# byronknoll/cmix

Hardware: AMD Instinct MI355X
Metric: input bytes/s on enwik8 at 1 GPU; compressed-size parity vs CPU ref (higher is better)
Workload: dtype f32

## Files before the change

cmix_amd/csrc/cmx_api.hip:

```cpp
#include <hip/hip_runtime.h>
#include <math.h>
#include <stdio.h>
#include <stdlib.h>
#include <string.h>
#include <stddef.h>
#include <string>
#include <map>
#include <mutex>
#include <vector>

#include "../../include/cmix_amd.h"
#include "mixnet_state.h"
#include "cmx_late.h"
#include "cmx_streams.h"
#include "cmx_verify.h"

extern "C" __global__ void cmx_mixnet_kernel(MixState*, const float*, const uint32_t*,
                                             const uint8_t*, const float*, int, float*, float*, int);
extern "C" __global__ void cmx_mixnet_spec_kernel(MixState*, SpecXfer*, const float*, const uint32_t*, const uint8_t*, const float*, int, float*,
                                                  float*, int);
extern "C" __global__ void cmx_mixnet_spec_jitter_kernel(MixState*, SpecXfer*, const float*, const uint32_t*, const uint8_t*, const float*, int, float*, float*, int);
extern "C" __global__ void cmx_mixnet_spec_late_kernel(MixState*, SpecXfer*, const float*, const uint32_t*, const float*, int, float*, float*, int, CmxLate);
extern "C" __global__ void cmx_mixnet_spec_verify_kernel(MixState*, SpecXfer*, const float*, const uint32_t*, const uint8_t*, const float*, int, float*, float*, int,
                                                         CmxVerify);
extern "C" __global__ void cmx_mixnet_verify_kernel(const MixState*, const float*, const uint32_t*, const uint8_t*, const float*, int, CmxVerify);
extern "C" __global__ void cmx_mixnet_verify_fold_kernel(CmxVerifyHdr*, unsigned long long, int);
extern "C" __global__ void cmx_mixnet_verify_xor_kernel(void*, int, unsigned);
extern "C" __global__ void cmx_sse_init_kernel(MixState*);
extern "C" __global__ void cmx_probe_libm_kernel(int, const float*, float*, size_t);

namespace {

thread_local std::string g_err;
void set_err(const std::string& s) { g_err = s; }

#define HIP_OK(call)                                                                  \
  do {                                                                                \
    hipError_t e_ = (call);                                                           \
    if (e_ != hipSuccess) {                                                           \
      set_err(std::string(#call) + ": " + hipGetErrorString(e_));                     \
      return fail_value;                                                              \
    }                                                                                 \
  } while (0)

const float kLr[CMX_MIXERS] = {
    0.005f, 0.0005f, 0.005f, 0.0005f, 0.005f, 0.002f, 0.002f, 0.005f, 0.00005f, 0.0007f, 0.0005f,
    0.002f, 0.0005f, 0.001f, 0.001f, 0.001f, 0.005f, 0.001f, 0.001f, 0.005f, 0.001f, 0.001f,
    0.005f, 0.005f, 0.005f, 0.003f,
    0.005f, 0.0005f, 0.005f, 0.0005f, 0.00001f, 0.005f, 0.005f, 0.005f, 0.0005f, 0.002f, 0.001f,
    0.001f, 0.001f, 0.001f, 0.001f, 0.001f, 0.001f, 0.001f, 0.001f, 0.001f,
    0.0003f};

#define CMX_MIXNET_THREADS 512
constexpr size_t kLdsBytes = (size_t)(17 * CMX_MIX0 * 68 + 2112 + 32 + 32 + 64 + 48 + 48 + 48) * 4;

void build_logit(std::vector<float>& t) {
  t.resize(100001);
  for (int i = 0; i < 100001; ++i) {
    float p = (i + 0.5f) / 100001;
    t[i] = logf(p / (1 - p));
  }
}

void build_sse_tables(std::vector<uint16_t>& t_st, std::vector<uint16_t>& t_sq) {
  const double LOG2E = 1.44269504088896340736;
  auto l2 = [&](double a) { return LOG2E * log(a); };
  auto e2 = [&](double a) { return exp(a / LOG2E); };
  auto st = [&](double p) { return l2((1 - p) / p); };
  auto sq = [&](double p) { return 1.0 / (1.0 + e2(p)); };
  const int SCALE = 32768, hSCALE = 16384;
  const double st_coef = (hSCALE - 1) / l2(SCALE - 1);
  const double sq_coef = 1.0 / st_coef;
  t_st.assign(SCALE, 0);
  t_sq.assign(SCALE, 0);
  for (int i = 1; i < SCALE; i++)
    t_sq[i] = (uint16_t)(unsigned)(sq((double)(i - hSCALE) * sq_coef) * SCALE);
  unsigned x = 0;
  for (unsigned i = 1; i < (unsigned)SCALE; i++) {
    unsigned s = (unsigned)(st((double)i / SCALE) * st_coef + hSCALE);
    t_st[i] = (uint16_t)s;
    if ((uint16_t)s != t_st[x]) {
      unsigned y = i - 1;
      t_sq[t_st[x]] = (uint16_t)((x + y + 1) / 2);
      x = i;
    }
  }
}

}

void cmx_set_err(const std::string& s) { set_err(s); }

struct cmx_mixnet {
  int device = 0;
  MixState* d_state = nullptr;
  MixState h_state;
  std::vector<void*> allocs;
  float* d_decay = nullptr;
  hipStream_t run_stream = nullptr; bool run_stream_set = false;
  hipStream_t s_up = nullptr; bool own_up = false;
  hipEvent_t ev_kdone[CMX_PIPELINE_SLOTS] = {};
  size_t decay_cap = 0;
  float* h_decay = nullptr;
  hipEvent_t ev_decay[CMX_PIPELINE_SLOTS] = {};
  bool decay_used[CMX_PIPELINE_SLOTS] = {};
  uint64_t runs = 0;
  uint64_t bits_done = 0;
  hipEvent_t ev0 = nullptr, ev1 = nullptr;
  bool timed = false;
  float* d_sync_probs = nullptr;
  uint32_t* d_sync_sel = nullptr;
  uint8_t* d_sync_bit = nullptr;
  float* d_sync_p = nullptr;
  float h_sync_decay = 0;
  bool predicted = false;
  const float* pend_probs = nullptr;
  const uint32_t* pend_sel = nullptr;
  unsigned char* h_sync_pin = nullptr;
  unsigned sync_slot = 0;
  int profile = 0;
  int dbg = 0;
  int rotate = 0;
  int jitter = 0;
  int xcd = -1;
  bool tolerance = false;
  SpecXfer* d_xfer = nullptr;
  float* d_late_p = nullptr; size_t late_p_cap = 0;
  float* late_mix_cur[3] = {nullptr, nullptr, nullptr};
  float* d_late_mix = nullptr;
  bool verify = false;
  CmxVerifyHdr* d_vhdr = nullptr;
  unsigned long long* d_vrec = nullptr; size_t vrec_blocks = 0;
  unsigned long long* d_vseg = nullptr;
  struct { int cls = 0; uint64_t bit = 0, index = 0; uint32_t mask = 0; } pert;
};

std::string cmx_mixnet_verify_text(const unsigned long long r[8]) {
  static const char* const names[CMX_VC_N] = {"?", "layer-0 row (raw inputs)", "coded bit", "selectors", "decay (gather wave)", "decay (tail-a wave)",
                                              "decay (tail-b wave)", "ring written (stretched inputs)", "ring read (stretched inputs)", "layer-0 row segment"};
  const unsigned cls = r[3] < CMX_VC_N ? (unsigned)r[3] : 0;
  std::string s = "verify mode: " + std::to_string(r[2]) + " mismatch(es) between what the mixing network consumed and its source; the first: " + names[cls] +
                  ", in the block of " + std::to_string(CMX_VERIFY_BLOCK) + " bits from stream bit " + std::to_string(r[4]);
  if (r[5] != ~0ull) s += ", mixer " + std::to_string(r[5]);
  if (r[6] != ~0ull) s += ", row " + std::to_string(r[6]);
  if (r[7] != ~0ull) s += ", segment " + std::to_string(r[7]);
  return s + " (the stream's output is void)";
}

extern "C" {

const char* cmx_last_error(void) { return g_err.c_str(); }
const char* cmx_version(void) { return "cmix_amd 0.1 (gfx950; cmix v21 predictor path)"; }

int cmx_device_count(void) {
  int n = 0;
  if (hipGetDeviceCount(&n) != hipSuccess) return 0;
  return n;
}


void* cmx_device_alloc(int device, size_t bytes) {
  void* p = nullptr;
  if (hipSetDevice(device) != hipSuccess || hipMalloc(&p, bytes ? bytes : 1) != hipSuccess) {
    set_err("cmx_device_alloc: hipMalloc failed");
    return nullptr;
  }
  return p;
}
void cmx_device_free(int device, void* p) {
  if (p && hipSetDevice(device) == hipSuccess) (void)hipFree(p);
}
void* cmx_host_alloc(size_t bytes) {
  void* p = nullptr;
  if (hipHostMalloc(&p, bytes ? bytes : 1, hipHostMallocDefault) != hipSuccess) { set_err("cmx_host_alloc: hipHostMalloc failed"); return nullptr; }
  return p;
}
void cmx_host_free(void* p) { if (p) (void)hipHostFree(p); }
void* cmx_late_alloc(size_t bytes) {
  void* p = nullptr;
  if (hipHostMalloc(&p, bytes ? bytes : 1, hipHostMallocMapped | hipHostMallocCoherent) != hipSuccess) { set_err("cmx_late_alloc: hipHostMalloc failed"); return nullptr; }
  memset(p, 0, bytes);
  return p;
}
void cmx_late_free(void* p) { if (p) (void)hipHostFree(p); }
void* cmx_late_alloc_dev(int device, size_t bytes) {
  void* p = nullptr;
  if (hipSetDevice(device) != hipSuccess) { set_err("cmx_late_alloc_dev: hipSetDevice failed"); return nullptr; }
  if (hipExtMallocWithFlags(&p, bytes ? bytes : 1, hipDeviceMallocUncached) != hipSuccess) {
    (void)hipGetLastError();
    if (hipExtMallocWithFlags(&p, bytes ? bytes : 1, hipDeviceMallocFinegrained) != hipSuccess) { set_err("cmx_late_alloc_dev: hipExtMallocWithFlags failed"); return nullptr; }
  }
  if (hipMemset(p, 0, bytes) != hipSuccess) { (void)hipFree(p); set_err("cmx_late_alloc_dev: hipMemset failed"); return nullptr; }
  return p;
}
void cmx_late_free_dev(void* p) { if (p) (void)hipFree(p); }
int cmx_copy_to_host(int device, void* dst, const void* d_src, size_t bytes) {
  if (hipSetDevice(device) != hipSuccess || hipDeviceSynchronize() != hipSuccess ||
      hipMemcpy(dst, d_src, bytes, hipMemcpyDeviceToHost) != hipSuccess) {
    set_err("cmx_copy_to_host: device error");
    return 1;
  }
  return 0;
}

void cmx_mixnet_destroy(cmx_mixnet_t* h) {
  if (!h) return;
  hipSetDevice(h->device);
  hipDeviceSynchronize();
  for (void* p : h->allocs) hipFree(p);
  if (h->h_decay) hipHostFree(h->h_decay);
  if (h->h_sync_pin) hipHostFree(h->h_sync_pin);
  if (h->ev0) hipEventDestroy(h->ev0);
  if (h->ev1) hipEventDestroy(h->ev1);
  for (int i = 0; i < CMX_PIPELINE_SLOTS; ++i) { if (h->ev_decay[i]) hipEventDestroy(h->ev_decay[i]); if (h->ev_kdone[i]) hipEventDestroy(h->ev_kdone[i]); }
  if (h->own_up && h->s_up) cmx_destroy_stream(h->s_up);
  delete h;
}

cmx_mixnet_t* cmx_mixnet_create(int device) {
  cmx_mixnet_t* const fail_value = nullptr;
  int n = cmx_device_count();
  if (n <= 0) { set_err("cmx_mixnet_create: no HIP device visible (a gfx950 GPU is required)"); return nullptr; }
  if (device < 0 || device >= n) { set_err("cmx_mixnet_create: bad device index"); return nullptr; }
  HIP_OK(hipSetDevice(device));
  hipDeviceProp_t prop;
  HIP_OK(hipGetDeviceProperties(&prop, device));
  if (!strstr(prop.gcnArchName, "gfx950")) {
    set_err(std::string("cmx_mixnet_create: device is ") + prop.gcnArchName + ", this library is built for gfx950 only");
    return nullptr;
  }
  cmx_mixnet_t* h = new cmx_mixnet();
  h->device = device;
  MixState& S = h->h_state;
  memset(&S, 0, sizeof S);
  auto dalloc = [&](size_t bytes, bool zero) -> void* {
    void* p = nullptr;
    if (hipMalloc(&p, bytes) != hipSuccess) return nullptr;
    h->allocs.push_back(p);
    if (zero) hipMemset(p, 0, bytes);
    return p;
  };
#define ALLOC(field, type, count, zero)                                       \
  do {                                                                        \
    S.field = (type*)dalloc((size_t)(count) * sizeof(type), zero);            \
    if (!S.field) { set_err("hipMalloc failed for " #field); cmx_mixnet_destroy(h); return nullptr; } \
  } while (0)
  std::vector<float> lut;
  std::vector<uint16_t> t_st, t_sq;
  build_logit(lut);
  build_sse_tables(t_st, t_sq);
  float* d_lut = (float*)dalloc(lut.size() * 4, false);
  uint16_t* d_st = (uint16_t*)dalloc(32768 * 2, false);
  uint16_t* d_sq = (uint16_t*)dalloc(32768 * 2, false);
  if (!d_lut || !d_st || !d_sq) { set_err("hipMalloc failed for tables"); cmx_mixnet_destroy(h); return nullptr; }
  hipMemcpy(d_lut, lut.data(), lut.size() * 4, hipMemcpyHostToDevice);
  hipMemcpy(d_st, t_st.data(), 32768 * 2, hipMemcpyHostToDevice);
  hipMemcpy(d_sq, t_sq.data(), 32768 * 2, hipMemcpyHostToDevice);
  S.logit_lut = d_lut;
  S.t_st = d_st;
  S.t_sq = d_sq;
  S.stretch_min = lut[0];
  S.stretch_max = lut[100000];
  memcpy(S.lr, kLr, sizeof kLr);
  ALLOC(rows0, float, (size_t)CMX_MIX0 * CMX_ROWS_PER_MIXER * CMX_ROW0_STRIDE, true);
  ALLOC(rows1, float, (size_t)CMX_MIX1 * CMX_ROWS_PER_MIXER * CMX_ROW1_STRIDE, true);
  ALLOC(rows2, float, (size_t)CMX_ROWS_PER_MIXER * CMX_ROW2_STRIDE, true);
  ALLOC(row_steps, uint64_t, (size_t)CMX_MIXERS * CMX_ROWS_PER_MIXER, true);
  ALLOC(map_keys, uint32_t, (size_t)CMX_MIXERS * CMX_MAP_SLOTS, true);
  ALLOC(map_vals, uint32_t, (size_t)CMX_MIXERS * CMX_MAP_SLOTS, true);
  ALLOC(s6, uint16_t, (size_t)CMX_SM6_VOL * 8, false);
  ALLOC(s7, uint16_t, (size_t)CMX_SM7_VOL * 8, false);
  ALLOC(x1, int, CMX_MIX1_VOL, false);
  ALLOC(x2, int, CMX_MIX2_VOL, false);
#undef ALLOC
  for (int i = 0; i <= CMX_MIXERS; ++i) S.max_steps[i] = 1;
  S.steps = 0;
  S.sse_j = 1;
  S.sse_pc = 0;
  S.sse_ffl = 0;
  for (int i = 0; i <= CMX_MIXERS; ++i) S.fwd_p[i] = 0.5f;
  h->d_state = (MixState*)dalloc(sizeof(MixState), false);
  if (!h->d_state) { set_err("hipMalloc failed for state"); cmx_mixnet_destroy(h); return nullptr; }
  hipMemcpy(h->d_state, &S, sizeof S, hipMemcpyHostToDevice);
  hipLaunchKernelGGL(cmx_sse_init_kernel, dim3(2048), dim3(256), 0, 0, h->d_state);
  h->d_sync_probs = (float*)dalloc(CMX_IN0 * 4, true);
  h->d_sync_sel = (uint32_t*)dalloc(CMX_MIXERS * 4, true);
  h->d_sync_bit = (uint8_t*)dalloc(16, true);
  h->d_sync_p = (float*)dalloc(16, true);
  if (hipFuncSetAttribute((const void*)cmx_mixnet_kernel, hipFuncAttributeMaxDynamicSharedMemorySize,
                          (int)kLdsBytes) != hipSuccess) {
    set_err("hipFuncSetAttribute(MaxDynamicSharedMemorySize) failed");
    cmx_mixnet_destroy(h);
    return nullptr;
  }
  h->d_xfer = (SpecXfer*)dalloc(sizeof(SpecXfer), true);
  bool attr_ok = true;
  for (const void* k : {(const void*)cmx_mixnet_spec_kernel, (const void*)cmx_mixnet_spec_jitter_kernel, (const void*)cmx_mixnet_spec_late_kernel,
                        (const void*)cmx_mixnet_spec_verify_kernel})
    attr_ok = attr_ok && hipFuncSetAttribute(k, hipFuncAttributeMaxDynamicSharedMemorySize, CMX_SPEC_LDS_BYTES) == hipSuccess;
  if (!h->d_xfer || !attr_ok) {
    set_err("cmx_mixnet_create: hand-off area / kernel attribute (spec kernel) failed");
    cmx_mixnet_destroy(h);
    return nullptr;
  }
  { const char* v = getenv("CMX_MIXNET_DBG"); h->dbg = v ? atoi(v) : 0; }
  { const char* v = getenv("CMX_MIXNET_JITTER"); h->jitter = v ? atoi(v) & 15 : 0; }
  { const char* v = getenv("CMX_MIXNET_ROTATE"); h->rotate = v && v[0] == '1'; }
  { const char* v = getenv("CMX_MIXNET_XCD"); h->xcd = v ? atoi(v) : CMX_MIXNET_XCD_DEFAULT; if (h->xcd > 7) h->xcd = -1; }
  hipEventCreate(&h->ev0);
  hipEventCreate(&h->ev1);
  for (int i = 0; i < CMX_PIPELINE_SLOTS; ++i) { hipEventCreateWithFlags(&h->ev_decay[i], hipEventDisableTiming); hipEventCreateWithFlags(&h->ev_kdone[i], hipEventDisableTiming); }
  hipError_t e = hipDeviceSynchronize();
  if (e != hipSuccess) { set_err(std::string("init: ") + hipGetErrorString(e)); cmx_mixnet_destroy(h); return nullptr; }
  return h;
}

static inline float decay_of(uint64_t steps) {
  return (float)(0.9 / pow(0.0000001 * steps + 0.8, 0.8));
}

static int ensure_decay(cmx_mixnet_t* h, size_t nbits) {
  const int fail_value = 1;
  if (nbits <= h->decay_cap) return 0;
  size_t cap = nbits < 4096 ? 4096 : nbits;
  if (h->h_decay) hipHostFree(h->h_decay);
  h->h_decay = nullptr;
  for (int i = 0; i < CMX_PIPELINE_SLOTS; ++i) {
    if (h->decay_used[i]) { (void)hipEventSynchronize(h->ev_decay[i]); (void)hipEventSynchronize(h->ev_kdone[i]); }
    h->decay_used[i] = false;
  }
  HIP_OK(hipHostMalloc((void**)&h->h_decay, (size_t)CMX_PIPELINE_SLOTS * cap * 4, hipHostMallocDefault));
  void* p = nullptr;
  HIP_OK(hipMalloc(&p, (size_t)CMX_PIPELINE_SLOTS * cap * 4));
  h->allocs.push_back(p);
  h->d_decay = (float*)p;
  h->decay_cap = cap;
  return 0;
}

int cmx_mixnet_spec_stats(cmx_mixnet_t* h, uint64_t out[5]) {
  const int fail_value = 1;
  if (!h || !out) { set_err("cmx_mixnet_spec_stats: bad argument"); return 1; }
  HIP_OK(hipSetDevice(h->device));
  HIP_OK(hipDeviceSynchronize());
  unsigned long long st[8];
  HIP_OK(hipMemcpy(st, (char*)h->d_xfer + offsetof(SpecXfer, stat), sizeof st, hipMemcpyDeviceToHost));
  for (int i = 0; i < 5; ++i) out[i] = st[i];
  return 0;
}

static bool g_cumask_applied = false;
static bool cumask_wanted() {
  static const char* const xe = getenv("CMX_MIXNET_XCD");
  static const bool w = getenv("CMX_CUMASK") != nullptr && xe && atoi(xe) >= 0 && atoi(xe) < 8 && getenv("CMX_PIPELINE_STREAMS") == nullptr;
  return w;
}
namespace {
std::mutex g_q_mu;
std::map<hipStream_t, int> g_q_dev;
int g_q_held[64];
}
int cmx_make_stream(hipStream_t* st, int which) {
  *st = nullptr;
  int dev = 0, cus = 0;
  if (hipGetDevice(&dev) != hipSuccess || hipDeviceGetAttribute(&cus, hipDeviceAttributeMultiprocessorCount, dev) != hipSuccess || cus <= 0 || cus > 32 * 32) {
    set_err("cmx_make_stream: no device"); return 1;
  }
  std::lock_guard<std::mutex> g(g_q_mu);
  int& held = g_q_held[dev & 63];
  if (held + 1 > CMX_MAX_HW_QUEUES) {
    set_err("cmx_make_stream: this process already holds " + std::to_string(held) + " dedicated hardware queues on device " + std::to_string(dev) + ", the limit is " +
            std::to_string(CMX_MAX_HW_QUEUES) + " (an engine takes 13, 14 when it decodes; CMX_PIPELINE_STREAMS=2 or 1 takes 8 or 6)");
    return 1;
  }
  const int words = (cus + 31) / 32;
  std::vector<uint32_t> full(words, 0u);
  for (int cu = 0; cu < cus; ++cu) full[cu / 32] |= 1u << (cu % 32);
  hipError_t e = hipErrorUnknown;
  if (cumask_wanted() && which != 2) {
    static const int x = atoi(getenv("CMX_MIXNET_XCD"));
    std::vector<uint32_t> m(words, 0u);
    for (int cu = 0; cu < cus; ++cu) if (((cu & 7) == x) == (which == 1)) m[cu / 32] |= 1u << (cu % 32);
    e = hipExtStreamCreateWithCUMask(st, (uint32_t)words, m.data());
    if (e == hipSuccess) { if (which == 1) g_cumask_applied = true; }
    else (void)hipGetLastError();
  }
  if (e != hipSuccess) e = hipExtStreamCreateWithCUMask(st, (uint32_t)words, full.data());
  if (e != hipSuccess) { *st = nullptr; set_err(std::string("cmx_make_stream: hipExtStreamCreateWithCUMask: ") + hipGetErrorString(e)); return 1; }
  g_q_dev[*st] = dev;
  ++held;
  return 0;
}
void cmx_destroy_stream(hipStream_t st) {
  if (!st) return;
  {
    std::lock_guard<std::mutex> g(g_q_mu);
    auto it = g_q_dev.find(st);
    if (it != g_q_dev.end()) { --g_q_held[it->second & 63]; g_q_dev.erase(it); }
  }
  (void)hipStreamDestroy(st);
}
int cmx_hw_queues(int device) {
  std::lock_guard<std::mutex> g(g_q_mu);
  return g_q_held[device & 63];
}

__global__ void cmx_overlap_probe_kernel(unsigned* cnt, unsigned* seen, int i, unsigned n, unsigned long long ticks) {
  if (threadIdx.x != 0) return;
  __hip_atomic_fetch_add(cnt, 1u, __ATOMIC_RELAXED, __HIP_MEMORY_SCOPE_AGENT);
  const unsigned long long t0 = wall_clock64();
  unsigned c = __hip_atomic_load(cnt, __ATOMIC_RELAXED, __HIP_MEMORY_SCOPE_AGENT);
  while (c < n && wall_clock64() - t0 < ticks) { __builtin_amdgcn_s_sleep(8); c = __hip_atomic_load(cnt, __ATOMIC_RELAXED, __HIP_MEMORY_SCOPE_AGENT); }
  __hip_atomic_store(seen + i, c, __ATOMIC_RELAXED, __HIP_MEMORY_SCOPE_AGENT);
}
int cmx_overlap_probe(const hipStream_t* st, int n, int* distinct) {
  std::vector<hipStream_t> q;
  for (int i = 0; i < n; ++i) {
    if (!st[i]) continue;
    bool dup = false;
// ... 96 lines not shown
}
int cmx_mixnet_mode(cmx_mixnet_t* h) { return h && h->tolerance ? 1 : 0; }

int cmx_mixnet_set_upload_stream(cmx_mixnet_t* h, void* stream) {
  if (!h) { set_err("cmx_mixnet_set_upload_stream: null handle"); return 1; }
  if (h->own_up && h->s_up) cmx_destroy_stream(h->s_up);
  h->s_up = (hipStream_t)stream; h->own_up = false;
  return 0;
}

static int mixnet_run_impl(cmx_mixnet_t* h, const float* d_probs, const uint32_t* d_sel, const uint8_t* d_bits, size_t nbits, float* d_p_out, float* d_mix_out,
                           void* stream, const CmxLate* box);
int cmx_mixnet_run(cmx_mixnet_t* h, const float* d_probs, const uint32_t* d_sel,
                   const uint8_t* d_bits, size_t nbits, float* d_p_out, float* d_mix_out,
                   void* stream) {
  return mixnet_run_impl(h, d_probs, d_sel, d_bits, nbits, d_p_out, d_mix_out, stream, nullptr);
}
int cmx_mixnet_run_late(cmx_mixnet_t* h, void* box, const float* probs, const uint32_t* sel, size_t nbits, void* stream) {
  if (!h || !box) { set_err("cmx_mixnet_run_late: bad argument"); return 1; }
  if (h->tolerance) { set_err("cmx_mixnet_run_late: a decoder needs the strict kernel (the tolerance switch is set)"); return 1; }
  if (h->verify) { set_err("cmx_mixnet_run_late: verify mode covers the compressor's kernel only"); return 1; }
  if (hipSetDevice(h->device) != hipSuccess) { set_err("hipSetDevice failed"); return 1; }
  if (h->late_p_cap < nbits || h->decay_cap < nbits) { set_err("cmx_mixnet_run_late: call cmx_mixnet_late_prepare first (nothing may be allocated while the stream's kernels run)"); return 1; }
  float* mix = h->d_late_mix ? h->d_late_mix + (size_t)(h->runs % 3) * h->late_p_cap * CMX_MIXERS : nullptr;
  h->late_mix_cur[h->runs % 3] = mix;
  return mixnet_run_impl(h, probs, sel, nullptr, nbits, h->d_late_p, mix, stream, (const CmxLate*)box);
}
int cmx_mixnet_late_prepare(cmx_mixnet_t* h, size_t nbits) {
  if (!h || !nbits) { set_err("cmx_mixnet_late_prepare: bad argument"); return 1; }
  if (h->verify) { set_err("cmx_mixnet_late_prepare: verify mode covers the compressor's kernel only"); return 1; }
  if (hipSetDevice(h->device) != hipSuccess) { set_err("hipSetDevice failed"); return 1; }
  if (h->late_p_cap < nbits) {
    void* p = nullptr;
    if (hipMalloc(&p, nbits * 4) != hipSuccess) { set_err("cmx_mixnet_late_prepare: hipMalloc failed"); return 1; }
    h->allocs.push_back(p);
    h->d_late_p = (float*)p; h->late_p_cap = nbits;
    const char* dbg = getenv("CMX_LATE_DEBUG");
    if (dbg && dbg[0] == '1') {
      if (hipMalloc(&p, 3 * nbits * CMX_MIXERS * 4) != hipSuccess) { set_err("cmx_mixnet_late_prepare: hipMalloc failed"); return 1; }
      h->allocs.push_back(p);
      h->d_late_mix = (float*)p;
    }
  }
  if (!h->s_up) { if (cmx_make_stream(&h->s_up, 2)) return 1; h->own_up = true; }
  return ensure_decay(h, nbits);
}
static int mixnet_run_impl(cmx_mixnet_t* h, const float* d_probs, const uint32_t* d_sel, const uint8_t* d_bits, size_t nbits, float* d_p_out, float* d_mix_out,
                           void* stream, const CmxLate* box) {
  const int fail_value = 1;
  if (!h) { set_err("cmx_mixnet_run: null handle"); return 1; }
  if (h->predicted) { set_err("cmx_mixnet_run: a bit-synchronous predict() is pending"); return 1; }
  if (nbits == 0) return 0;
  if (nbits > 0x7fffffff) { set_err("cmx_mixnet_run: chunk too large"); return 1; }
  HIP_OK(hipSetDevice(h->device));
  hipStream_t st = (hipStream_t)stream;
  if (h->run_stream_set && st != h->run_stream) { set_err("cmx_mixnet_run: every chunk of a handle must be enqueued on the same stream"); return 1; }
  h->run_stream = st; h->run_stream_set = true;
  if (ensure_decay(h, nbits)) return 1;
  if (!h->s_up) { if (cmx_make_stream(&h->s_up, 2)) return 1; h->own_up = true; }
  const size_t vblocks = (nbits + CMX_VERIFY_BLOCK - 1) / CMX_VERIFY_BLOCK;
  if (!box && h->verify) {
    if (h->pert.cls && h->pert.cls != CMX_VC_SEGMENT && h->pert.bit >= nbits) { set_err("cmx_mixnet_run: the armed verify perturbation lies outside the chunk"); return 1; }
    if (vblocks > h->vrec_blocks) {
      HIP_OK(hipStreamSynchronize(st));
      if (h->d_vrec) { for (auto& a : h->allocs) if (a == h->d_vrec) a = nullptr; (void)hipFree(h->d_vrec); h->d_vrec = nullptr; }
      const size_t nb = vblocks < 512 ? 512 : vblocks;
      void* a = nullptr;
      HIP_OK(hipMalloc(&a, nb * CMX_VERIFY_REC * 8));
      h->allocs.push_back(a);
      h->d_vrec = (unsigned long long*)a; h->vrec_blocks = nb;
    }
  }
  const int slot = (int)(h->runs++ % CMX_PIPELINE_SLOTS);
  if (h->decay_used[slot]) HIP_OK(hipEventSynchronize(h->ev_kdone[slot]));
  float* hd = h->h_decay + (size_t)slot * h->decay_cap;
  float* dd = h->d_decay + (size_t)slot * h->decay_cap;
  for (size_t t = 0; t < nbits; ++t) hd[t] = decay_of(h->bits_done + t);
  HIP_OK(hipMemcpyAsync(dd, hd, nbits * 4, hipMemcpyHostToDevice, h->s_up));
  HIP_OK(hipEventRecord(h->ev_decay[slot], h->s_up));
  HIP_OK(hipStreamWaitEvent(st, h->ev_decay[slot], 0));
  h->decay_used[slot] = true;
  HIP_OK(hipEventRecord(h->ev0, st));
  HIP_OK(hipMemsetAsync(h->d_xfer, 0, CMX_SPEC_HEADER_BYTES, st));
  const bool cumask = cmx_cumask_on() != 0;
  const int rot = h->rotate && h->xcd < 0 ? (int)((h->runs * 3) & 7) : 0;
  const int kmode = 3 | (rot << 8) | (h->profile ? 4 : 0) | ((h->dbg & 15) << 4) | (h->tolerance ? 0x1000 : 0) | (h->xcd >= 0 ? 0x20000 | ((h->xcd & 7) << 20) : 0) |
                    (getenv("CMX_MIXNET_XCD_NOLOCAL") ? 0x800000 : 0) | (cumask ? 0x1000000 : 0) | (h->jitter ? 0x2000000 | ((h->jitter & 15) << 26) : 0);
  static const bool padgrid = getenv("CMX_MIXNET_PADGRID") != nullptr;
  const unsigned grid = (1 + CMX_SPEC_HELPERS) * ((h->xcd >= 0 && !cumask) || padgrid ? 8 : 1) + (unsigned)rot;
  if (box && box->box)
    hipLaunchKernelGGL(cmx_mixnet_spec_late_kernel, dim3(grid), dim3(CMX_SPEC_THREADS), CMX_SPEC_LDS_BYTES, st,
                       h->d_state, h->d_xfer, d_probs, d_sel, dd, (int)nbits, d_p_out, d_mix_out, kmode, *box);
  else if (h->verify) {
    HIP_OK(hipMemsetAsync(h->d_vhdr, 0, CMX_VERIFY_CLEAR_BYTES, st));
    HIP_OK(hipMemsetAsync(h->d_vrec, 0, vblocks * CMX_VERIFY_REC * 8, st));
    const auto p = h->pert;
    h->pert.cls = 0;
    void* pw = nullptr; int pbytes = 4;
    if (p.cls == CMX_VC_ROW) pw = (void*)(d_probs + p.bit * CMX_IN0 + p.index);
    else if (p.cls == CMX_VC_SEL) pw = (void*)(d_sel + p.bit * CMX_MIXERS + p.index);
    else if (p.cls == CMX_VC_BIT) { pw = (void*)(d_bits + p.bit); pbytes = 1; }
    else if (p.cls == CMX_VC_DECAY_GATHER || p.cls == CMX_VC_DECAY_TAIL_A || p.cls == CMX_VC_DECAY_TAIL_B) pw = (void*)(dd + p.bit);
    if (p.cls == CMX_VC_SEGMENT)
      hipLaunchKernelGGL(cmx_mixnet_verify_xor_kernel, dim3(1), dim3(64), 0, st, (void*)(h->h_state.rows0 + p.bit * CMX_ROW0_STRIDE + p.index), 4, p.mask);
    const bool ring = p.cls == CMX_VC_RING_WRITTEN || p.cls == CMX_VC_RING_READ;
    const CmxVerify V = {h->d_vrec, h->d_vseg, h->d_vhdr, ring ? (int)p.bit : -1, ring ? (int)p.index : 0, ring ? p.mask : 0u};
    hipLaunchKernelGGL(cmx_mixnet_spec_verify_kernel, dim3(grid), dim3(CMX_SPEC_THREADS), CMX_SPEC_LDS_BYTES, st,
                       h->d_state, h->d_xfer, d_probs, d_sel, d_bits, dd, (int)nbits, d_p_out, d_mix_out, kmode, V);
    HIP_OK(hipGetLastError());
    if (pw) hipLaunchKernelGGL(cmx_mixnet_verify_xor_kernel, dim3(1), dim3(64), 0, st, pw, pbytes, p.mask);
    hipLaunchKernelGGL(cmx_mixnet_verify_kernel, dim3((unsigned)vblocks), dim3(256), 0, st, (const MixState*)h->d_state, d_probs, d_sel, d_bits, (const float*)dd, (int)nbits, V);
    if (pw) hipLaunchKernelGGL(cmx_mixnet_verify_xor_kernel, dim3(1), dim3(64), 0, st, pw, pbytes, p.mask);
    hipLaunchKernelGGL(cmx_mixnet_verify_fold_kernel, dim3(1), dim3(64), 0, st, h->d_vhdr, (unsigned long long)h->bits_done, (int)nbits);
  } else {
    hipLaunchKernelGGL(h->jitter ? cmx_mixnet_spec_jitter_kernel : cmx_mixnet_spec_kernel, dim3(grid), dim3(CMX_SPEC_THREADS), CMX_SPEC_LDS_BYTES, st,
                       h->d_state, h->d_xfer, d_probs, d_sel, d_bits, dd, (int)nbits, d_p_out, d_mix_out, kmode);
  }
  HIP_OK(hipGetLastError());
  HIP_OK(hipEventRecord(h->ev_kdone[slot], st));
  HIP_OK(hipEventRecord(h->ev1, st));
  h->timed = true;
  h->bits_done += nbits;
  return 0;
}

float cmx_mixnet_predict(cmx_mixnet_t* h, const float* probs, const uint32_t* sel) {
  const float fail_value = -1.0f;
  if (!h) { set_err("cmx_mixnet_predict: null handle"); return -1.0f; }
  if (h->predicted) { set_err("cmx_mixnet_predict: called twice without perceive()"); return -1.0f; }
  if (h->verify) { set_err("cmx_mixnet_predict: verify mode covers chunks only (the bit-synchronous kernel writes rows it does not digest)"); return -1.0f; }
  HIP_OK(hipSetDevice(h->device));
  HIP_OK(hipMemcpy(h->d_sync_probs, probs, CMX_IN0 * 4, hipMemcpyHostToDevice));
  HIP_OK(hipMemcpy(h->d_sync_sel, sel, CMX_MIXERS * 4, hipMemcpyHostToDevice));
  hipLaunchKernelGGL(cmx_mixnet_kernel, dim3(1), dim3(CMX_MIXNET_THREADS), kLdsBytes, 0, h->d_state,
                     h->d_sync_probs, h->d_sync_sel, h->d_sync_bit, h->d_decay, 1, h->d_sync_p,
                     (float*)nullptr, 1);
  HIP_OK(hipGetLastError());
  float p = -1.0f;
  HIP_OK(hipMemcpy(&p, h->d_sync_p, 4, hipMemcpyDeviceToHost));
  h->predicted = true;
  return p;
}

int cmx_mixnet_perceive(cmx_mixnet_t* h, int bit) {
  const int fail_value = 1;
  if (!h) { set_err("cmx_mixnet_perceive: null handle"); return 1; }
  if (!h->predicted) { set_err("cmx_mixnet_perceive: no pending predict()"); return 1; }
  HIP_OK(hipSetDevice(h->device));
  if (ensure_decay(h, 1)) return 1;
  uint8_t b = bit ? 1 : 0;
  float d = decay_of(h->bits_done);
  HIP_OK(hipMemcpy(h->d_sync_bit, &b, 1, hipMemcpyHostToDevice));
  HIP_OK(hipMemcpy(h->d_decay, &d, 4, hipMemcpyHostToDevice));
  hipLaunchKernelGGL(cmx_mixnet_kernel, dim3(1), dim3(CMX_MIXNET_THREADS), kLdsBytes, 0, h->d_state,
                     h->d_sync_probs, h->d_sync_sel, h->d_sync_bit, h->d_decay, 1, h->d_sync_p,
                     (float*)nullptr, 2);
  HIP_OK(hipGetLastError());
  HIP_OK(hipDeviceSynchronize());
  h->predicted = false;
  h->bits_done += 1;
  return 0;
}

int cmx_mixnet_predict_async(cmx_mixnet_t* h, const float* d_probs, const uint32_t* d_sel, float* d_p, void* stream) {
  const int fail_value = 1;
  if (!h || !d_probs || !d_sel || !d_p) { set_err("cmx_mixnet_predict_async: bad argument"); return 1; }
  if (h->predicted) { set_err("cmx_mixnet_predict_async: called twice without perceive()"); return 1; }
  if (h->verify) { set_err("cmx_mixnet_predict_async: verify mode covers chunks only"); return 1; }
  HIP_OK(hipSetDevice(h->device));
  hipLaunchKernelGGL(cmx_mixnet_kernel, dim3(1), dim3(CMX_MIXNET_THREADS), kLdsBytes, (hipStream_t)stream, h->d_state,
                     d_probs, d_sel, h->d_sync_bit, (const float*)(h->d_sync_bit + 4), 1, d_p, (float*)nullptr, 1);
  HIP_OK(hipGetLastError());
  h->pend_probs = d_probs;
  h->pend_sel = d_sel;
  h->predicted = true;
  return 0;
}

int cmx_mixnet_perceive_async(cmx_mixnet_t* h, int bit, void* stream) {
  const int fail_value = 1;
  if (!h) { set_err("cmx_mixnet_perceive_async: null handle"); return 1; }
  if (!h->predicted || !h->pend_probs) { set_err("cmx_mixnet_perceive_async: no pending predict_async()"); return 1; }
  HIP_OK(hipSetDevice(h->device));
  if (!h->h_sync_pin) HIP_OK(hipHostMalloc((void**)&h->h_sync_pin, 16 * 8, hipHostMallocDefault));
  unsigned char* slot = h->h_sync_pin + 8 * (h->sync_slot++ & 15);
  slot[0] = bit ? 1 : 0;
  const float d = decay_of(h->bits_done);
  memcpy(slot + 4, &d, 4);
  hipStream_t st = (hipStream_t)stream;
  HIP_OK(hipMemcpyAsync(h->d_sync_bit, slot, 8, hipMemcpyHostToDevice, st));
  hipLaunchKernelGGL(cmx_mixnet_kernel, dim3(1), dim3(CMX_MIXNET_THREADS), kLdsBytes, st, h->d_state, h->pend_probs,
                     h->pend_sel, h->d_sync_bit, (const float*)(h->d_sync_bit + 4), 1, h->d_sync_p, (float*)nullptr, 2);
  HIP_OK(hipGetLastError());
  h->predicted = false;
  h->pend_probs = nullptr;
  h->bits_done += 1;
  return 0;
}
// ... 76 lines not shown
```

cmix_amd/csrc/lstm_api.hip:

```cpp
#include <hip/hip_runtime.h>
#include <math.h>
#include <stddef.h>
#include <stdio.h>
#include <stdlib.h>
#include <string.h>
#include <string>
#include <vector>

#include "../../include/cmix_amd.h"
#include "mixnet_state.h"
#include "lstm_state.h"
#include "cmx_late.h"
#include "cmx_glibc_rand.h"

extern "C" __global__ void cmx_lstm_prep(const LstmState, const float*, const uint8_t*, size_t, int, int);
extern "C" __global__ void cmx_lstm_bptt_acc(const LstmState, int, int, int, int);
extern "C" __global__ void cmx_lstm_bptt_gb(const LstmState, int, int);
extern "C" __global__ void cmx_lstm_bptt_acc_mfma(const LstmState, int, int);
extern "C" __global__ void cmx_lstm_fwdblk(const LstmState, const uint8_t*, const float*, float*, size_t, int, int, int);
extern "C" __global__ void cmx_lstm_fwdblk_late(const LstmState, CmxLate, const float*, const float*, float*, int, int, int, int, int);
extern "C" __global__ void cmx_lstm_bpttblk(const LstmState);
extern "C" __global__ void cmx_bytemodel_bits(const float*, const float*, const uint8_t*, size_t, float*, int*, size_t, int,
                                              float*);
extern "C" __global__ void cmx_bytemodel_late_kernel(CmxLate, size_t, const float*, const float*, const float*, const float*, const float*, const uint32_t*, uint32_t,
                                                     const uint32_t*, uint32_t, float*, size_t, int16_t*, uint8_t*, uint8_t*, const cmx_late_relay_t*, int);

void cmx_set_err(const std::string& s);


struct cmx_lstm {
  int device = 0;
  LstmState h_state;
  std::vector<void*> allocs;
  float* d_prev_probs = nullptr;
  uint64_t bytes_done = 0;
  int hc = 0;
  size_t fb_lds = 0, bp_lds = 0;
  uint64_t bptt_rounds = 0;
  bool tolerance = false;
};


extern "C" {

void cmx_lstm_destroy(cmx_lstm_t* h) {
  if (!h) return;
  (void)hipSetDevice(h->device);
  (void)hipDeviceSynchronize();
  for (void* p : h->allocs) (void)hipFree(p);
  delete h;
}

int cmx_glibc_rand_selftest(uint32_t seed, int n, int* out) {
  GlibcRand g(seed);
  for (int i = 0; i < n; ++i) out[i] = g.next();
  return 0;
}

cmx_lstm_t* cmx_lstm_create(const uint8_t vocab[256], int skip_rand, int device) {
  int ndev = cmx_device_count();
  if (ndev <= 0) { cmx_set_err("cmx_lstm_create: no HIP device visible (a gfx950 GPU is required)"); return nullptr; }
  if (device < 0 || device >= ndev) { cmx_set_err("cmx_lstm_create: bad device index"); return nullptr; }
  if (hipSetDevice(device) != hipSuccess) { cmx_set_err("hipSetDevice failed"); return nullptr; }
  cmx_lstm_t* h = new cmx_lstm();
  h->device = device;
  LstmState& S = h->h_state;
  memset(&S, 0, sizeof S);
  int V = 0;
  for (int i = 0; i < 256; ++i) {
    S.vocab[i] = vocab[i] != 0;
    S.byte_map[i] = V;
    if (S.vocab[i]) ++V;
  }
  if (V == 0) { cmx_set_err("cmx_lstm_create: empty vocabulary"); delete h; return nullptr; }
  S.V = V;
  S.insz[0] = 1 + LSTM_C + V;
  S.insz[1] = V + 1 + 2 * LSTM_C;
  S.rowlen[0] = S.insz[0] + V;
  S.rowlen[1] = S.insz[1] + V;
  S.lr = 0.03f;
  { const char* v = getenv("CMX_LSTM_XCD"); S.xcd = v ? atoi(v) : -1; }
  { const char* v = getenv("CMX_LSTM_AVOID_XCD"); if (!v) v = getenv("CMX_MIXNET_XCD"); S.avoid_xcd = v ? atoi(v) : CMX_MIXNET_XCD_DEFAULT; if (S.avoid_xcd > 7) S.avoid_xcd = -1; }
  bool fail = false;
  auto dallocf = [&](size_t count, const float* init) -> float* {
    void* p = nullptr;
    if (hipMalloc(&p, count * 4) != hipSuccess) { fail = true; return nullptr; }
    h->allocs.push_back(p);
    if (init) (void)hipMemcpy(p, init, count * 4, hipMemcpyHostToDevice);
    else (void)hipMemset(p, 0, count * 4);
    return (float*)p;
  };
  GlibcRand rng(0xDEADBEEFu);
  for (int i = 0; i < skip_rand; ++i) rng.next();
  for (int l = 0; l < LSTM_L; ++l) {
    const int rl = S.rowlen[l];
    std::vector<float> w[3], wt[3];
    for (int g = 0; g < 3; ++g) { w[g].resize((size_t)LSTM_C * rl); wt[g].resize((size_t)LSTM_C * rl); }
    const float val = sqrtf(6.0f / (float)(V + V));
    const float low = -val, range = 2 * val;
    for (int i = 0; i < LSTM_C; ++i) {
      for (int j = 0; j < rl; ++j)
        for (int g = 0; g < 3; ++g) w[g][(size_t)i * rl + j] = low + ((float)rng.next() / (float)2147483647) * range;
      w[0][(size_t)i * rl + rl - 1] = 1;
    }
    for (int g = 0; g < 3; ++g) {
      for (int i = 0; i < LSTM_C; ++i)
        for (int j = 0; j < rl; ++j) wt[g][lstm_wt_index(V, S.insz[l], j, i)] = w[g][(size_t)i * rl + j];
      S.W[l][g] = dallocf((size_t)LSTM_C * rl, w[g].data());
      S.WT[l][g] = dallocf((size_t)LSTM_C * rl, wt[g].data());
      S.M[l][g] = dallocf((size_t)LSTM_C * rl, nullptr);
      S.Vv[l][g] = dallocf((size_t)LSTM_C * rl, nullptr);
      std::vector<float> gb(8 * LSTM_C, 0.0f);
      for (int i = 0; i < LSTM_C; ++i) gb[i] = 1.0f;
      S.gb[l][g] = dallocf(8 * LSTM_C, gb.data());
      S.norm[l][g] = dallocf((size_t)LSTM_H * LSTM_C, nullptr);
      S.gstate[l][g] = dallocf((size_t)LSTM_H * LSTM_C, nullptr);
      S.ivar[l][g] = dallocf(LSTM_H, nullptr);
      S.raw[l][g] = dallocf(LSTM_C, nullptr);
      S.E[l][g] = dallocf((size_t)LSTM_H * LSTM_C, nullptr);
    }
    S.last_state[l] = dallocf((size_t)LSTM_H * LSTM_C, nullptr);
    S.tanh_state[l] = dallocf((size_t)LSTM_H * LSTM_C, nullptr);
    S.in_gate_state[l] = dallocf((size_t)LSTM_H * LSTM_C, nullptr);
    S.state[l] = dallocf(LSTM_C, nullptr);
    S.stateb[0][l] = S.state[l];
    S.stateb[1][l] = dallocf(LSTM_C, nullptr);
    std::vector<float> li((size_t)LSTM_H * S.insz[l], 0.0f);
    for (int e = 0; e < LSTM_H; ++e) li[(size_t)e * S.insz[l] + S.insz[l] - 1] = 1.0f;
    S.layer_input[l] = dallocf(li.size(), li.data());
  }
  S.OL = dallocf((size_t)LSTM_H * V * LSTM_NH, nullptr);
  S.OLT = nullptr;
  {
    std::vector<float> out((size_t)LSTM_H * LSTM_VP, 0.0f);
    for (int e = 0; e < LSTM_H; ++e)
      for (int i = 0; i < V; ++i) out[(size_t)e * LSTM_VP + i] = (float)(1.0 / V);
    S.output = dallocf(out.size(), out.data());
  }
  {
    std::vector<float> hid(LSTM_NH, 0.0f);
    hid[LSTM_NH - 1] = 1.0f;
    S.hid[0] = dallocf(LSTM_NH, hid.data());
    S.hid[1] = dallocf(LSTM_NH, hid.data());
  }
  S.input_history = (unsigned*)dallocf(LSTM_H, nullptr);
  S.bp_symbol = (unsigned*)dallocf(LSTM_H, nullptr);
  S.logits = dallocf(LSTM_VP, nullptr);
  {
    std::vector<float> tab(4 * (LSTM_UPDATE_LIMIT + 1), 0.0f);
    const float beta1 = 0.025f, beta2 = 0.9999f, lr = S.lr;
    const unsigned long long limit = LSTM_UPDATE_LIMIT;
    for (unsigned long long s = 0; s <= limit; ++s) {
      float t = (float)s, alpha, b1, b2;
      if (t < limit) {
        alpha = lr * 0.1f / sqrtf(5e-5f * t + 1.0f);
        b1 = (float)(1.0f - powf(beta1, t));
        b2 = (float)(1.0f - powf(beta2, t));
      } else {
        alpha = lr * 0.1f / sqrtf(5e-5f * limit + 1.0f);
        b1 = (float)(1.0f - pow(beta1, limit));
        b2 = (float)(1.0f - pow(beta2, limit));
      }
      tab[4 * s] = alpha;
      tab[4 * s + 1] = b1;
      tab[4 * s + 2] = b2;
    }
    S.adam_tab = dallocf(tab.size(), tab.data());
  }
  {
    std::vector<float> bp(256, (float)(1.0 / 256));
    S.byte_probs = dallocf(256, bp.data());
    h->d_prev_probs = dallocf(256, bp.data());
  }
  S.dyn = (int*)dallocf(4, nullptr);
  S.sync = (LstmSync*)dallocf((sizeof(LstmSync) + 3) / 4, nullptr);
  S.raw_ring = dallocf((size_t)LSTM_L * LSTM_H * 3 * LSTM_C, nullptr);
  S.h_ring = dallocf((size_t)LSTM_H * LSTM_NH, nullptr);
  S.logit_ring = dallocf((size_t)LSTM_H * LSTM_VP, nullptr);
  S.bp_pub = dallocf((size_t)2 * LSTM_H * 2 * LSTM_C, nullptr);
  {
    const size_t nq1 = (size_t)(S.insz[1] + 3) / 4;
    const size_t gate = nq1 * LSTM_FB_R * 16 + (836 + 3 * LSTM_C + 4 + 256) * 4;
    const size_t ro = (size_t)(V + LSTM_FB_GO - 1) / LSTM_FB_GO, rp = ro | 1;
    const size_t outl = (size_t)((LSTM_NH + 3) / 4) * rp * 16 + (2 * 404 + 256 + 256 + 36 + 36 + 4) * 4;
    h->fb_lds = gate > outl ? gate : outl;
    h->bp_lds = (size_t)9 * 50 * LSTM_BP_J * 16 +
                ((size_t)3 * 256 * LSTM_BP_J + 3 * 256 + 3 * LSTM_C + 3 * LSTM_C + 4 + 6 * LSTM_BP_J) * 4;
    if (hipFuncSetAttribute((const void*)cmx_lstm_fwdblk, hipFuncAttributeMaxDynamicSharedMemorySize, (int)h->fb_lds) != hipSuccess ||
        hipFuncSetAttribute((const void*)cmx_lstm_fwdblk_late, hipFuncAttributeMaxDynamicSharedMemorySize, (int)h->fb_lds) != hipSuccess ||
        hipFuncSetAttribute((const void*)cmx_lstm_bpttblk, hipFuncAttributeMaxDynamicSharedMemorySize, (int)h->bp_lds) != hipSuccess)
      fail = true;
  }
  S.blk = (LstmBlockArgs*)dallocf((sizeof(LstmBlockArgs) + 3) / 4 + 4, nullptr);
  if (fail) {
    cmx_set_err("cmx_lstm_create: hipMalloc failed");
    cmx_lstm_destroy(h);
    return nullptr;
  }
  if (hipDeviceSynchronize() != hipSuccess) { cmx_set_err("cmx_lstm_create: init failed"); cmx_lstm_destroy(h); return nullptr; }
  return h;
}

int cmx_lstm_vocab_size(const cmx_lstm_t* h) { return h ? h->h_state.V : -1; }

int cmx_lstm_run(cmx_lstm_t* h, const float* d_in_probs, const uint8_t* d_bytes, size_t nbytes,
                 float* d_out_probs, float* d_bit_p, size_t bit_p_stride, int* d_bit_ex, void* stream) {
  if (!h) { cmx_set_err("cmx_lstm_run: null handle"); return 1; }
  if (nbytes == 0) return 0;
  if (hipSetDevice(h->device) != hipSuccess) { cmx_set_err("hipSetDevice failed"); return 1; }
  hipStream_t st = (hipStream_t)stream;
  const LstmState& S = h->h_state;
  const int V = S.V;
  if (d_bit_p) (void)hipMemcpyAsync(h->d_prev_probs, S.byte_probs, 256 * 4, hipMemcpyDeviceToDevice, st);
  if (!d_in_probs) { cmx_set_err("cmx_lstm_run: d_in_probs is required"); return 1; }
  auto sync_reset = [&]() {
    return hipMemsetAsync((char*)S.sync + 16, 0, sizeof(LstmSync) - 16, st) == hipSuccess;
  };
  for (size_t n = 0; n < nbytes;) {
    const int e = (int)(h->bytes_done % LSTM_H);
    const int hc = h->hc;
    int us = 0;
    if (e == 0) {
      h->bptt_rounds += 1;
      us = (int)(h->bptt_rounds < LSTM_UPDATE_LIMIT ? h->bptt_rounds : LSTM_UPDATE_LIMIT);
    }
    if (e == 0) {
      hipLaunchKernelGGL(cmx_lstm_prep, dim3(1), dim3(256), 0, st, S, d_in_probs + n * 256, d_bytes, n, e, -1);
      if (!sync_reset()) { cmx_set_err("cmx_lstm_run: hipMemsetAsync failed"); return 1; }
      hipLaunchKernelGGL(cmx_lstm_bpttblk, dim3(lstm_grid_for_roles(LSTM_BP_G, S.avoid_xcd)), dim3(LSTM_BP_THREADS), h->bp_lds, st, S);
      if (h->tolerance) hipLaunchKernelGGL(cmx_lstm_bptt_acc_mfma, dim3((S.rowlen[1] + 15) / 16, (LSTM_C + 15) / 16, 6), dim3(64), 0, st, S, us, -1);
      else { const int gx = (S.rowlen[1] + 63) / 64, gy = LSTM_C / 4; hipLaunchKernelGGL(cmx_lstm_bptt_acc, dim3(lstm_grid_for_roles(gx * gy * 6, S.avoid_xcd)), dim3(64, 4), 0, st, S, us, -1, gx, gy); }
      hipLaunchKernelGGL(cmx_lstm_bptt_gb, dim3(6), dim3(256), 0, st, S, us, -1);
    }
    const size_t left = nbytes - n;
    const int cnt = (int)(left < (size_t)(LSTM_H - e) ? left : (size_t)(LSTM_H - e));
    if (!sync_reset()) { cmx_set_err("cmx_lstm_run: hipMemsetAsync failed"); return 1; }
    hipLaunchKernelGGL(cmx_lstm_fwdblk, dim3(lstm_grid_for_roles(2 * LSTM_FB_GL + LSTM_FB_GO, S.avoid_xcd)), dim3(LSTM_FB_THREADS), h->fb_lds, st, S, d_bytes,
                       d_in_probs, d_out_probs, n, cnt, e, hc);
    h->hc ^= 1;
    h->bytes_done += cnt;
    n += cnt;
  }
  if (d_bit_p) {
    if (!d_out_probs) { cmx_set_err("cmx_lstm_run: bit predictions need d_out_probs"); return 1; }
    hipLaunchKernelGGL(cmx_bytemodel_bits, dim3((unsigned)nbytes), dim3(64), 0, st, h->d_prev_probs, d_out_probs,
                       d_bytes, nbytes, d_bit_p, d_bit_ex, bit_p_stride ? bit_p_stride : (size_t)1, -1, (float*)nullptr);
  }
  hipError_t e = hipGetLastError();
  if (e != hipSuccess) { cmx_set_err(std::string("cmx_lstm_run: ") + hipGetErrorString(e)); return 1; }
  return 0;
}

int cmx_lstm_run_late(cmx_lstm_t* h, const void* late_box, const float* d_ppmd, const float* h_ppmd, const uint8_t* h_bytes, float* d_out, size_t b0, size_t nchunk, void* stream) {
  if (!h || !late_box || !d_ppmd || !h_ppmd || !h_bytes || !d_out || b0 >= nchunk) { cmx_set_err("cmx_lstm_run_late: bad argument"); return -1; }
  if (hipSetDevice(h->device) != hipSuccess) { cmx_set_err("hipSetDevice failed"); return -1; }
  if (h->tolerance) { cmx_set_err("cmx_lstm_run_late: a decoder is strict"); return -1; }
  hipStream_t st = (hipStream_t)stream;
  const LstmState& S = h->h_state;
  const int e = (int)(h->bytes_done % LSTM_H);
  const int hc = h->hc;
  auto sync_reset = [&]() { return hipMemsetAsync((char*)S.sync + 16, 0, sizeof(LstmSync) - 16, st) == hipSuccess; };
  if (e == 0) {
    h->bptt_rounds += 1;
    const int us = (int)(h->bptt_rounds < LSTM_UPDATE_LIMIT ? h->bptt_rounds : LSTM_UPDATE_LIMIT);
    hipLaunchKernelGGL(cmx_lstm_prep, dim3(1), dim3(256), 0, st, S, h_ppmd + (b0 + 1) * 256, h_bytes, b0, e, -1);
    if (!sync_reset()) { cmx_set_err("cmx_lstm_run_late: hipMemsetAsync failed"); return -1; }
    hipLaunchKernelGGL(cmx_lstm_bpttblk, dim3(lstm_grid_for_roles(LSTM_BP_G, S.avoid_xcd)), dim3(LSTM_BP_THREADS), h->bp_lds, st, S);
    { const int gx = (S.rowlen[1] + 63) / 64, gy = LSTM_C / 4; hipLaunchKernelGGL(cmx_lstm_bptt_acc, dim3(lstm_grid_for_roles(gx * gy * 6, S.avoid_xcd)), dim3(64, 4), 0, st, S, us, -1, gx, gy); }
    hipLaunchKernelGGL(cmx_lstm_bptt_gb, dim3(6), dim3(256), 0, st, S, us, -1);
  }
  const size_t left = nchunk - b0;
  const int cnt = (int)(left < (size_t)(LSTM_H - e) ? left : (size_t)(LSTM_H - e));
  if (!sync_reset()) { cmx_set_err("cmx_lstm_run_late: hipMemsetAsync failed"); return -1; }
  hipLaunchKernelGGL(cmx_lstm_fwdblk_late, dim3(lstm_grid_for_roles(2 * LSTM_FB_GL + LSTM_FB_GO, S.avoid_xcd)), dim3(LSTM_FB_THREADS), h->fb_lds, st, S, *(const CmxLate*)late_box,
                     d_ppmd, h_ppmd, d_out, (int)b0, cnt, e, hc, (int)nchunk);
  h->hc ^= 1;
  h->bytes_done += cnt;
  const hipError_t er = hipGetLastError();
  if (er != hipSuccess) { cmx_set_err(std::string("cmx_lstm_run_late: ") + hipGetErrorString(er)); return -1; }
  return cnt;
}

int cmx_lstm_set_tolerance(cmx_lstm_t* h, int on) {
  if (!h) { cmx_set_err("cmx_lstm_set_tolerance: null handle"); return 1; }
  if (h->bytes_done && h->tolerance != (on != 0)) { cmx_set_err("cmx_lstm_set_tolerance: only before the first byte (a stream is strict or tolerant from its start)"); return 1; }
  h->tolerance = on != 0;
  return 0;
}
int cmx_lstm_failed(cmx_lstm_t* h) {
  if (!h) return 1;
  (void)hipSetDevice(h->device);
  if (hipDeviceSynchronize() != hipSuccess) return 1;
  unsigned f = 0;
  if (hipMemcpy(&f, &h->h_state.sync->fail, 4, hipMemcpyDeviceToHost) != hipSuccess) return 1;
  return f ? 1 : 0;
}

const unsigned* cmx_lstm_fail_flag(cmx_lstm_t* h) { return h ? &h->h_state.sync->fail : nullptr; }

int cmx_bytemodel_bits_run(int device, const float* d_dist0, const float* d_dist_rest, const uint8_t* d_bytes,
                           size_t nbytes, float* d_bit_p, size_t bit_p_stride, int* d_bit_ex, void* stream) {
  if (nbytes == 0) return 0;
  if (hipSetDevice(device) != hipSuccess) { cmx_set_err("hipSetDevice failed"); return 1; }
  hipLaunchKernelGGL(cmx_bytemodel_bits, dim3((unsigned)nbytes), dim3(64), 0, (hipStream_t)stream, d_dist0,
                     d_dist_rest, d_bytes, nbytes, d_bit_p, d_bit_ex, bit_p_stride ? bit_p_stride : (size_t)1, -1,
                     (float*)nullptr);
  hipError_t e = hipGetLastError();
  if (e != hipSuccess) { cmx_set_err(std::string("cmx_bytemodel_bits_run: ") + hipGetErrorString(e)); return 1; }
  return 0;
}

int cmx_bytemodel_late_run(int device, void* box, size_t nbytes, const float* brk0, const float* brk, const float* ppmd, const float* lstm0, const float* lstm,
                           const uint32_t* c0_brk, uint32_t c0_brk_want, const uint32_t* c0_lstm, uint32_t c0_lstm_want, float* layer0, size_t pstride,
                           int16_t* hint_pr, uint8_t* hint_ex, uint8_t* dbit0, const void* relay_dev, int nrelay, void* stream) {
  if (!box || !nbytes || !brk0 || !brk || !ppmd || !lstm0 || !lstm || !layer0 || !hint_pr || !hint_ex || !dbit0 || nrelay < 0 || nrelay > CMX_LATE_RELAY_MAX || (nrelay && !relay_dev)) {
    cmx_set_err("cmx_bytemodel_late_run: bad argument");
    return 1;
  }
  if (hipSetDevice(device) != hipSuccess) { cmx_set_err("hipSetDevice failed"); return 1; }
  hipLaunchKernelGGL(cmx_bytemodel_late_kernel, dim3(1), dim3(192 + 64 * 6), 0, (hipStream_t)stream, *(const CmxLate*)box, nbytes, brk0, brk, ppmd, lstm0, lstm, c0_brk, c0_brk_want,
                     c0_lstm, c0_lstm_want, layer0, pstride, hint_pr, hint_ex, dbit0, (const cmx_late_relay_t*)relay_dev, nrelay);
  hipError_t e = hipGetLastError();
  if (e != hipSuccess) { cmx_set_err(std::string("cmx_bytemodel_late_run: ") + hipGetErrorString(e)); return 1; }
  return 0;
}
const float* cmx_lstm_byte_probs(cmx_lstm_t* h) { return h ? h->h_state.byte_probs : nullptr; }

int cmx_bytemodel_bit_run(int device, const float* d_dist, const uint8_t* d_byte, int k, float* d_bit_p,
                          size_t bit_p_stride, int* d_bit_ex, float* d_p_copy, void* stream) {
  if (!d_dist || !d_byte || !d_bit_p || k < 0 || k > 7) { cmx_set_err("cmx_bytemodel_bit_run: bad argument"); return 1; }
  if (hipSetDevice(device) != hipSuccess) { cmx_set_err("hipSetDevice failed"); return 1; }
  hipLaunchKernelGGL(cmx_bytemodel_bits, dim3(1), dim3(64), 0, (hipStream_t)stream, d_dist, d_dist, d_byte, (size_t)1,
                     d_bit_p, d_bit_ex, bit_p_stride ? bit_p_stride : (size_t)1, k, d_p_copy);
  hipError_t e = hipGetLastError();
  if (e != hipSuccess) { cmx_set_err(std::string("cmx_bytemodel_bit_run: ") + hipGetErrorString(e)); return 1; }
  return 0;
}

int cmx_lstm_get_gate_weights(cmx_lstm_t* h, int layer, int gate, float* out) {
  if (!h) return 1;
  (void)hipSetDevice(h->device);
  (void)hipDeviceSynchronize();
  size_t n = (size_t)LSTM_C * h->h_state.rowlen[layer];
  return hipMemcpy(out, h->h_state.W[layer][gate], n * 4, hipMemcpyDeviceToHost) == hipSuccess ? 0 : 1;
}
int cmx_lstm_gate_rowlen(const cmx_lstm_t* h, int layer) { return h ? h->h_state.rowlen[layer] : -1; }

}
```

cmix_amd/csrc/lstm_block.hip:

```cpp
#include <hip/hip_runtime.h>
#include <stdint.h>
#include "cmx_libm.h"
#include "lstm_state.h"
#include "cmx_late.h"

namespace {

__device__ __forceinline__ float fmul(float a, float b) { return __fmul_rn(a, b); }
__device__ __forceinline__ float fadd(float a, float b) { return __fadd_rn(a, b); }
__device__ __forceinline__ float fsub(float a, float b) { return __fsub_rn(a, b); }
__device__ __forceinline__ float fdiv(float a, float b) { return __fdiv_rn(a, b); }
__device__ __forceinline__ float fsqrt(float a) { return __builtin_sqrtf(a); }

constexpr int C = LSTM_C, H = LSTM_H, NH = LSTM_NH, VP = LSTM_VP;
constexpr int GL = LSTM_FB_GL, R = LSTM_FB_R, GO = LSTM_FB_GO, FT = LSTM_FB_THREADS;
constexpr int GB = LSTM_BP_G, J = LSTM_BP_J, BT = LSTM_BP_THREADS;
constexpr unsigned SPIN_LIMIT = 1u << 23;

__device__ __forceinline__ unsigned ld_u(const unsigned* p) { return __hip_atomic_load(p, __ATOMIC_RELAXED, __HIP_MEMORY_SCOPE_AGENT); }
__device__ __forceinline__ float ld_f(const float* p) { return __hip_atomic_load(p, __ATOMIC_RELAXED, __HIP_MEMORY_SCOPE_AGENT); }
__device__ __forceinline__ void st_f(float* p, float v) { __hip_atomic_store(p, v, __ATOMIC_RELAXED, __HIP_MEMORY_SCOPE_AGENT); }

__device__ __forceinline__ void lds_barrier() { asm volatile("s_waitcnt lgkmcnt(0)\n\ts_barrier" ::: "memory"); }

// ... 281 lines not shown
      const float err = (i0 + tid == cur_sym) ? fsub(o, 1.0f) : o;
      le_s[tid] = fmul(S->lr, err);
    }
    lds_barrier();
    for (int idx = tid; idx < nr * NQ; idx += FT) {
      const int rr = idx / NQ, q = idx - rr * NQ, j = q * 4;
      const float le = le_s[rr];
      float4 v = OLs[(size_t)q * RP + rr];
      float* dst = S->OL + ((size_t)e * V + i0 + rr) * NH + j;
      v.x = fsub(v.x, fmul(le, hprev[j]));
      dst[0] = v.x;
      if (j + 3 < NH) {
        v.y = fsub(v.y, fmul(le, hprev[j + 1]));
        v.z = fsub(v.z, fmul(le, hprev[j + 2]));
        v.w = fsub(v.w, fmul(le, hprev[j + 3]));
        dst[1] = v.y; dst[2] = v.z; dst[3] = v.w;
      }
      OLs[(size_t)q * RP + rr] = v;
    }
    wg_wait_t<LATE>(&Y->h_flag[0][e], 1, &Y->fail, LB);
    if (tid < C) hcur[tid] = ld_f(&S->h_ring[(size_t)e * NH + tid]);
    lds_barrier();
    float sum = 0.0f;
    if (tid < 64) sum = lds_chain(sum, OLs, RP, r, hcur, 0, C);
    wg_wait_t<LATE>(&Y->h_flag[1][e], 1, &Y->fail, LB);
    if (tid < C) hcur[C + tid] = ld_f(&S->h_ring[(size_t)e * NH + C + tid]);
    if (tid == 0) hcur[2 * C] = 1.0f;
    lds_barrier();
    if (tid < 64) {
      sum = lds_chain(sum, OLs, RP, r, hcur, C, NH);
      if (tid < nr) st_f(&S->logit_ring[(size_t)e * VP + i0 + tid], sum);
      wave_signal(&Y->logit_cnt[e]);
    }
    wg_wait_t<LATE>(&Y->logit_cnt[e], GO, &Y->fail, LB);
    float lg = 0.0f;
    if (tid < V) lg = ld_f(&S->logit_ring[(size_t)e * VP + tid]);
    red[tid] = tid < V ? lg : 0.0f;
    lds_barrier();
    for (int s = 128; s > 0; s >>= 1) {
      if (tid < s) red[tid] = fmaxf(red[tid], red[tid + s]);
      lds_barrier();
    }
    const float mx = red[0];
    if (tid < V) lgs[tid] = cmx_expf(fsub(lg, mx));
    lds_barrier();
    if (tid == 0) {
      float t = 0.0f;
#pragma unroll 16
      for (int i = 0; i < V; ++i) t = fadd(t, lgs[i]);
      tot_s[0] = t;
    }
    lds_barrier();
    float p = 0.0f;
    if (tid < V) p = fdiv(lgs[tid], tot_s[0]);
    lds_barrier();
    if (tid < V) {
      lgs[tid] = p;
      if (lead) S->output[(size_t)e * VP + tid] = p;
    }
    lds_barrier();
    if (tid < nr) outp[tid] = lgs[i0 + tid];
    if (lead) {
      const float pbv = S->vocab[tid] ? lgs[S->byte_map[tid]] : 0.0f;
      S->byte_probs[tid] = pbv;
      if (A.out_probs) A.out_probs[n * 256 + tid] = pbv;
    }
    if (LATE && lead) {
      asm volatile("s_waitcnt vmcnt(0)" ::: "memory");
      __syncthreads();
      if (tid == 0 && !ld_u(&Y->fail)) { late_publish(A.late, LC_LSTM, (uint32_t)(n + 1)); late_stamp(A.late, 9); }
    }
    pb ^= 1;
  }
}

}

extern "C" __global__ __launch_bounds__(LSTM_FB_THREADS) void cmx_lstm_fwdblk(const LstmState P, const uint8_t* bytes,
                                                                             const float* in_probs, float* out_probs,
                                                                             size_t n0, int cnt, int e0, int hc) {
  extern __shared__ float4 fb_lds[];
  FbArgs A;
  A.bytes = bytes; A.in_probs = in_probs; A.out_probs = out_probs; A.n0 = n0; A.cnt = cnt; A.e0 = e0; A.hc = hc;
  const int b = lstm_role_of_block((int)blockIdx.x, P.avoid_xcd);
  if (b < 0 || b >= 2 * GL + GO) return;
  A.late = CmxLate(); A.d_ppmd = nullptr; A.h_ppmd = nullptr; A.nchunk = 0;
  if (b < GL) fb_gate_wg<false>(&P, A, 0, b, reinterpret_cast<float*>(fb_lds));
  else if (b < 2 * GL) fb_gate_wg<false>(&P, A, 1, b - GL, reinterpret_cast<float*>(fb_lds));
  else fb_out_wg<false>(&P, A, b - 2 * GL, reinterpret_cast<float*>(fb_lds));
}

extern "C" __global__ __launch_bounds__(LSTM_FB_THREADS) void cmx_lstm_fwdblk_late(const LstmState P, CmxLate late, const float* d_ppmd, const float* h_ppmd,
                                                                                  float* out_probs, int b0, int cnt, int e0, int hc, int nchunk) {
  extern __shared__ float4 fb_lds[];
  FbArgs A;
  A.bytes = nullptr; A.in_probs = nullptr; A.out_probs = out_probs; A.n0 = (size_t)b0; A.cnt = cnt; A.e0 = e0; A.hc = hc;
  A.late = late; A.d_ppmd = d_ppmd; A.h_ppmd = h_ppmd; A.nchunk = nchunk;
  const int b = lstm_role_of_block((int)blockIdx.x, P.avoid_xcd);
  if (b < 0 || b >= 2 * GL + GO) return;
  if (b < GL) fb_gate_wg<true>(&P, A, 0, b, reinterpret_cast<float*>(fb_lds));
  else if (b < 2 * GL) fb_gate_wg<true>(&P, A, 1, b - GL, reinterpret_cast<float*>(fb_lds));
  else fb_out_wg<true>(&P, A, b - 2 * GL, reinterpret_cast<float*>(fb_lds));
}

namespace {
struct BpItem {
  int g, c; bool on;
  float gam_c, gam_o, gu_c, gu_o, bu_c, bu_o;
  float norm, iv, err;
};
}

extern "C" __global__ __launch_bounds__(LSTM_BP_THREADS) void cmx_lstm_bpttblk(const LstmState P) {
  extern __shared__ float4 bp_lds[];
  const LstmState* S = &P;
  LstmSync* Y = S->sync;
  const int tid = threadIdx.x, V = S->V, b = lstm_role_of_block((int)blockIdx.x, P.avoid_xcd), j0 = b * J;
  if (b < 0 || b >= GB) return;
  const bool lead = b == 0;
  float4* Wb = bp_lds;
  float* olb = reinterpret_cast<float*>(Wb + 9 * 50 * J);
  float* errs = olb + 3 * 256 * J;
  float* gerr = errs + 3 * 256;
  float* gprod = gerr + 3 * C;
  float* gsm = gprod + 3 * C;
  float* fres = gsm + 4;
  for (int idx = tid; idx < 9 * 50 * J; idx += BT) {
    const int slot = idx / (50 * J), rem = idx - slot * 50 * J, q = rem / J, cl = rem - q * J;
    const int layer = slot < 3 ? 0 : 1, gg = slot % 3, kind = slot >= 6 ? 1 : 0;
    const int rl = S->rowlen[layer];
    const float* wsrc = S->W[layer][gg] + 2 * V + kind * C + j0 + cl;
    float4 v;
    v.x = wsrc[(size_t)(4 * q) * rl]; v.y = wsrc[(size_t)(4 * q + 1) * rl];
    v.z = wsrc[(size_t)(4 * q + 2) * rl]; v.w = wsrc[(size_t)(4 * q + 3) * rl];
    Wb[idx] = v;
  }
  float stored_c = 0.0f, stored_o = 0.0f, serr_c = 0.0f, serr_o = 0.0f;
  BpItem ia, ib;
  auto item_init = [&](BpItem& it, int idx) {
    it.on = idx < 3 * C;
    const int id = it.on ? idx : 0;
    it.g = id / C; it.c = id - it.g * C;
    it.gam_o = S->gb[0][it.g][it.c]; it.gam_c = S->gb[1][it.g][it.c];
    it.gu_c = it.gu_o = it.bu_c = it.bu_o = 0.0f;
    it.norm = it.iv = it.err = 0.0f;
  };
  item_init(ia, tid);
  item_init(ib, BT + tid);
  constexpr int NSL = (256 * J + BT - 1) / BT;
  float olr[NSL];
  float errr = 0.0f;
  auto slice_load = [&](int s) {
    const int epoch = H - 1 - (s >> 1), layer = 1 - (s & 1);
#pragma unroll
    for (int u = 0; u < NSL; ++u) {
      const int idx = tid + u * BT, i = idx / J, cl = idx - i * J;
      olr[u] = i < V ? S->OL[((size_t)epoch * V + i) * NH + layer * C + j0 + cl] : 0.0f;
    }
    if (tid < V) {
      const float o = S->output[(size_t)epoch * VP + tid];
      errr = ((unsigned)tid == S->input_history[epoch]) ? fsub(o, 1.0f) : o;
    }
  };
  auto slice_store = [&](int s) {
    float* ob = olb + (s % 3) * 256 * J;
#pragma unroll
    for (int u = 0; u < NSL; ++u) {
      const int idx = tid + u * BT;
      if (idx < 256 * J) ob[idx] = olr[u];
    }
    if (tid < V) errs[(s % 3) * 256 + tid] = errr;
  };
  auto p1_chain = [&](int s, float h) -> float {
    const float* ob = olb + (s % 3) * 256 * J + (tid < J ? tid : 0);
    const float* ev = errs + (s % 3) * 256;
    int i = 0;
    for (; i + 8 <= V; i += 8) {
      float a[8], x[8];
#pragma unroll
      for (int k = 0; k < 8; ++k) { a[k] = ob[(i + k) * J]; x[k] = ev[i + k]; }
#pragma unroll
      for (int k = 0; k < 8; ++k) h = fadd(h, fmul(a[k], x[k]));
    }
    for (; i < V; ++i) h = fadd(h, fmul(ob[i * J], ev[i]));
    return h;
  };
  slice_load(0); slice_store(0);
  slice_load(1); slice_store(1);
  slice_load(2);
  lds_barrier();
  float* pub = S->bp_pub;
  if (tid < 64) {
    const float h = p1_chain(0, 0.0f);
    if (tid < J) { st_f(pub + j0 + tid, h); st_f(pub + C + j0 + tid, 0.0f); }
    wave_signal(&Y->bp_cnt[0]);
  }
  float hpre = 0.0f;
#pragma unroll 1
  for (int s = 0; s < 2 * H; ++s) {
    const int epoch = H - 1 - (s >> 1), layer = 1 - (s & 1);
    if (s + 2 < 2 * H) slice_store(s + 2);
// ... 114 lines not shown
```

cmix_amd/csrc/lstm_kernels.hip:

```cpp
#include <hip/hip_runtime.h>
#include <stdint.h>
#include "cmx_libm.h"
#include "lstm_state.h"
#include "cmx_late.h"

namespace {

__device__ __forceinline__ float fmul(float a, float b) { return __fmul_rn(a, b); }
__device__ __forceinline__ float fadd(float a, float b) { return __fadd_rn(a, b); }
__device__ __forceinline__ float fsub(float a, float b) { return __fsub_rn(a, b); }
__device__ __forceinline__ float fdiv(float a, float b) { return __fdiv_rn(a, b); }
__device__ __forceinline__ float fsqrt(float a) { return __builtin_sqrtf(a); }

constexpr int C = LSTM_C, H = LSTM_H, NH = LSTM_NH, VP = LSTM_VP;

}

__device__ __forceinline__ void lstm_prep(const LstmState* S, const float* in256, const uint8_t* bytes, size_t n, int e) {
  const int tid = threadIdx.x, V = S->V;
  if (S->vocab[tid]) {
    float v = fmul(in256[tid], 2.0f);
    int k = S->byte_map[tid];
    S->layer_input[0][(size_t)e * S->insz[0] + k] = v;
    S->layer_input[1][(size_t)e * S->insz[1] + k] = v;
  }
  if (tid == 0) {
    int sym = S->byte_map[bytes[n]];
    int last = e == 0 ? H - 1 : e - 1;
    S->dyn[0] = (int)S->input_history[last];
    S->input_history[last] = (unsigned)sym;
  }
  (void)V;
}

extern "C" __global__ void cmx_lstm_prep(const LstmState P, const float* in256, const uint8_t* bytes, size_t n, int e, int k) {
  if (k >= 0) { const LstmBlockArgs a = *P.blk; in256 = a.in_probs + a.n0 * 256; bytes = a.bytes; n = a.n0; e = 0; }
  lstm_prep(&P, in256, bytes, n, e);
}

extern "C" __global__ void cmx_lstm_bptt_acc(const LstmState P, int update_steps, int k, int gx, int gy) {
  const LstmState* S = &P;
  if (k >= 0) update_steps = P.blk->us;
  __shared__ float es[H][4];
  __shared__ float ins[H][64];
  __shared__ unsigned sym[H];
  const int role = lstm_role_of_block((int)blockIdx.x, P.avoid_xcd);
  if (role < 0 || role >= gx * gy * 6) return;
  const int bx = role % gx, by = (role / gx) % gy, bz = role / (gx * gy);
  const int layer = bz / 3, g = bz % 3;
  const int V = S->V, rl = S->rowlen[layer], insz = S->insz[layer];
  const int c = bx * 64 + threadIdx.x, i = by * 4 + threadIdx.y;
  const int t = threadIdx.y * 64 + threadIdx.x;
  for (int k = t; k < H * 4; k += 256) es[k >> 2][k & 3] = S->E[layer][g][(size_t)(k >> 2) * C + by * 4 + (k & 3)];
  for (int k = t; k < H * 64; k += 256) {
    int ee = k >> 6, cc = bx * 64 + (k & 63);
    ins[ee][k & 63] = (cc >= V && cc < rl) ? S->layer_input[layer][(size_t)ee * insz + (cc - V)] : 0.0f;
  }
  if (t < H) sym[t] = S->bp_symbol[t];
  __syncthreads();
  if (c >= rl) return;
  float acc = 0.0f;
  if (c < V) {
    for (int e = H - 1; e >= 0; --e)
      if (sym[e] == (unsigned)c) acc = fadd(acc, es[e][threadIdx.y]);
  } else {
    for (int e = H - 1; e >= 0; --e) acc = fadd(acc, fmul(es[e][threadIdx.y], ins[e][threadIdx.x]));
  }
  const float* tab = S->adam_tab + 4 * update_steps;
  const float alpha = tab[0], b1 = tab[1], b2 = tab[2];
  const float beta1 = 0.025f, beta2 = 0.9999f, eps = 1e-6f;
  const size_t ix = (size_t)i * rl + c;
  float m = S->M[layer][g][ix], v = S->Vv[layer][g][ix], w = S->W[layer][g][ix];
  m = fmul(m, beta1);
  m = fadd(m, fmul(fsub(1.0f, beta1), acc));
  v = fmul(v, beta2);
  v = fadd(v, fmul(fmul(fsub(1.0f, beta2), acc), acc));
  w = fsub(w, fmul(alpha, fdiv(fdiv(m, b1), fsqrt(fadd(fdiv(v, b2), eps)))));
  S->M[layer][g][ix] = m;
  S->Vv[layer][g][ix] = v;
  S->W[layer][g][ix] = w;
  S->WT[layer][g][lstm_wt_index(V, insz, c, i)] = w;
}

extern "C" __global__ __launch_bounds__(64) void cmx_lstm_bptt_acc_mfma(const LstmState P, int update_steps, int k) {
  const LstmState* S = &P;
  if (k >= 0) update_steps = P.blk->us;
  typedef float f32x4 __attribute__((ext_vector_type(4)));
  const int layer = blockIdx.z / 3, g = blockIdx.z % 3;
  const int V = S->V, rl = S->rowlen[layer], insz = S->insz[layer];
  const int lane = threadIdx.x, c0 = blockIdx.x * 16, i0 = blockIdx.y * 16;
  const int am = i0 + (lane & 15), bn = c0 + (lane & 15), kk = lane >> 4;
  const float* E = S->E[layer][g];
  const float* LI = S->layer_input[layer];
  const bool aval = am < C, bval = bn >= V && bn < rl;
  f32x4 acc = {0.0f, 0.0f, 0.0f, 0.0f};
  for (int e0 = 0; e0 < H; e0 += 4) {
    const int e = e0 + kk;
    const float a = (aval && e < H) ? E[(size_t)e * C + am] : 0.0f;
    const float b = (bval && e < H) ? LI[(size_t)e * insz + (bn - V)] : 0.0f;
    acc = __builtin_amdgcn_mfma_f32_16x16x4f32(a, b, acc, 0, 0, 0);
  }
  const int c = bn;
  if (c >= rl) return;
  const float* tab = S->adam_tab + 4 * update_steps;
  const float alpha = tab[0], b1 = tab[1], b2 = tab[2];
  const float beta1 = 0.025f, beta2 = 0.9999f, eps = 1e-6f;
  for (int r = 0; r < 4; ++r) {
    const int i = i0 + 4 * kk + r;
    if (i >= C) continue;
    float a_ = acc[r];
    if (c < V) {
      a_ = 0.0f;
      for (int e = H - 1; e >= 0; --e) if (S->bp_symbol[e] == (unsigned)c) a_ = fadd(a_, E[(size_t)e * C + i]);
    }
    const size_t ix = (size_t)i * rl + c;
    float m = S->M[layer][g][ix], v = S->Vv[layer][g][ix], w = S->W[layer][g][ix];
    m = fmul(m, beta1);
    m = fadd(m, fmul(fsub(1.0f, beta1), a_));
    v = fmul(v, beta2);
    v = fadd(v, fmul(fmul(fsub(1.0f, beta2), a_), a_));
    w = fsub(w, fmul(alpha, fdiv(fdiv(m, b1), fsqrt(fadd(fdiv(v, b2), eps)))));
    S->M[layer][g][ix] = m;
    S->Vv[layer][g][ix] = v;
    S->W[layer][g][ix] = w;
    S->WT[layer][g][lstm_wt_index(V, insz, c, i)] = w;
  }
}

extern "C" __global__ void cmx_lstm_bptt_gb(const LstmState P, int update_steps, int k) {
  const LstmState* S = &P;
// ... 143 lines not shown
```

cmix_amd/csrc/lstm_state.h:

```cpp
#ifndef CMX_LSTM_STATE_H
#define CMX_LSTM_STATE_H
#include <stdint.h>

#define LSTM_C 200
#define LSTM_L 2
#define LSTM_H 100
#define LSTM_NH 401
#define LSTM_VP 256
#define LSTM_UPDATE_LIMIT 3000
#define LSTM_FB_GL 12
#define LSTM_FB_R 50
#define LSTM_FB_GO 8
#define LSTM_FB_THREADS 256
#define LSTM_BP_G 20
#define LSTM_BP_J 10
#define LSTM_BP_THREADS 512

struct LstmSync {
  unsigned fail;
  unsigned pad[3];
  unsigned raw_cnt[LSTM_L][LSTM_H];
  unsigned h_flag[LSTM_L][LSTM_H];
  unsigned logit_cnt[LSTM_H];
  unsigned bp_cnt[2 * LSTM_H];
};

struct LstmBlockArgs {
  const float* in_probs;
  const unsigned char* bytes;
  float* out_probs;
  unsigned long long n0;
  int hc0;
  int us;
};

struct LstmState {
  int V;
  int insz[LSTM_L];
  int rowlen[LSTM_L];
  int* dyn;
  struct LstmBlockArgs* blk;
  int byte_map[256];
  unsigned char vocab[256];
  float lr;
  int xcd;
  int avoid_xcd;

  float* W[LSTM_L][3];
  float* WT[LSTM_L][3];
  float* M[LSTM_L][3];
  float* Vv[LSTM_L][3];
  float* gb[LSTM_L][3];
  float* norm[LSTM_L][3];
  float* gstate[LSTM_L][3];
  float* ivar[LSTM_L][3];
  float* last_state[LSTM_L];
  float* tanh_state[LSTM_L];
  float* in_gate_state[LSTM_L];
  float* state[LSTM_L];
  float* stateb[2][LSTM_L];
  float* layer_input[LSTM_L];
  float* OL;
  float* OLT;
  float* output;
  float* hid[2];
  unsigned* input_history;
  unsigned* bp_symbol;
  float* raw[LSTM_L][3];
  float* logits;
  float* E[LSTM_L][3];
  const float* adam_tab;
  float* byte_probs;
  struct LstmSync* sync;
  float* raw_ring;
  float* h_ring;
  float* logit_ring;
  float* bp_pub;
};

#if defined(__HIPCC__) || defined(__cplusplus)
static inline
#if defined(__HIPCC__)
__host__ __device__
#endif
int lstm_role_of_block(int b, int avoid) {
  if (avoid < 0) return b;
  if ((b & 7) == avoid) return -1;
  return b - (b >= avoid ? (b - avoid) / 8 + 1 : 0);
}
static inline int lstm_grid_for_roles(int n, int avoid) {
  if (avoid < 0) return n;
  int g = n;
  while (lstm_role_of_block(g - 1, avoid) < n - 1) ++g;
  return g;
}
static inline
#if defined(__HIPCC__)
__host__ __device__
#endif
size_t lstm_wt_index(int V, int insz, int c, int i) {
  if (c < V) return (size_t)c * LSTM_C + i;
  const int d = c - V, full = insz & ~3;
  if (d < full) return (size_t)V * LSTM_C + ((size_t)(d >> 2) * LSTM_C + i) * 4 + (d & 3);
  return (size_t)V * LSTM_C + (size_t)full * LSTM_C + (size_t)(d - full) * LSTM_C + i;
}
#endif

#endif
```

cmix_amd/csrc/mixnet_chunk.hip:

```cpp
#include "mixnet_dev.h"
#include "cmx_late.h"
#include "cmx_verify.h"

namespace {

constexpr int SEG = 548;
constexpr unsigned SPIN_LIMIT = 1u << 27;

struct Ctl {
  int staged[2];
  int consumed;
  int u_epoch;
  int scout_epoch;
  int tail_in;
  int tail_done;
  int abort;
  int b_in, b_done;
  int bit_epoch;
  unsigned late_lo, late_hi;
};

struct BitRec {
  uint32_t rowidx[48];
  uint32_t changed[32];
  float aux3[4];
  float lstm_p;
  int bit;
  uint32_t auxkey;
  int pad;
};

struct TailRec {
  float out0[32];
  float aux3[4];
  uint32_t rowidx[24];
  float lstm_p;
  int bit;
  int pad[2];
};

struct Lds {
  BitRec* rec;
  int rr;
  int lead;
  TailRec* trec;
  float* upd;
  uint32_t* dflag;
  float* in2;
  Ctl* ctl;
  float* w2;
  float* w1;
  unsigned pfdump;
  uint64_t* exptab;
  const uint16_t* lst;
  const uint16_t* lsq;
  int* sdone;
  float* h2;
  int* bitring;
  CmxLate late;
  int jit;
};

template <bool JIT> __device__ __forceinline__ void jitter_stall(int jit, int t, int who) {
  if constexpr (!JIT) return;
  unsigned h = (unsigned)t * 2654435761u + (unsigned)who * 0x9E3779B9u + (unsigned)jit * 0x85EBCA6Bu;
  h ^= h >> 15; h *= 0x2C1B3C6Du; h ^= h >> 12;
  if ((h & 7u) == 0) {
    const int n = (int)((h >> 3) & 31u);
    for (int i = 0; i < n; ++i) __builtin_amdgcn_s_sleep(127);
  }
}

__device__ __forceinline__ unsigned long long wave_sum_u64(unsigned long long v) {
#pragma unroll
  for (int o = 32; o > 0; o >>= 1) v += __shfl_xor(v, o, 64);
  return v;
}
__device__ __forceinline__ void verify_flag(const CmxVerify& V, unsigned long long key) {
  atomicAdd(&V.hdr->launch_count, 1ull);
  atomicMax(&V.hdr->launch_first, ~key);
}

typedef __attribute__((address_space(3))) int lds_int;
__device__ __forceinline__ int lds_poll(const int* p) {
  int v;
  asm volatile("ds_read_b32 %0, %1\n\ts_waitcnt lgkmcnt(0)" : "=v"(v) : "v"((const lds_int*)p) : "memory");
  return v;
}
__device__ __forceinline__ void lds_publish_store(int* p, int v) {
  asm volatile("s_waitcnt lgkmcnt(0)\n\tds_write_b32 %0, %1" :: "v"((lds_int*)p), "v"(v) : "memory");
}
__device__ __forceinline__ void touch_line(gptr<const float> g, unsigned lds_dst) {
  unsigned keep;
  const unsigned dst = __builtin_amdgcn_readfirstlane(lds_dst);
  asm volatile("s_mov_b32 %0, m0\n\ts_mov_b32 m0, %2\n\ts_nop 0\n\tglobal_load_lds_dword %1, off\n\ts_mov_b32 m0, %0"
               : "=&s"(keep) : "v"(g), "s"(dst) : "memory");
}
__device__ __forceinline__ void st_rel(int* p, int v) { lds_publish_store(p, v); }
__device__ __forceinline__ CmxLateBox* ctl_box(Ctl* ctl) {
  const unsigned lo = (unsigned)lds_poll((const int*)&ctl->late_lo), hi = (unsigned)lds_poll((const int*)&ctl->late_hi);
  return reinterpret_cast<CmxLateBox*>(((unsigned long long)hi << 32) | lo);
}
__device__ __forceinline__ bool late_expired(CmxLateBox* B, unsigned long long& t0) {
  if (late_ld(&B->abort) || late_ld(&B->fail)) return true;
  const unsigned long long now = wall_clock64();
  if (!t0) { t0 = now; return false; }
  if (now - t0 > late_timeout_ticks(B)) { late_st(&B->fail, 1u); return true; }
  return false;
}
template <bool LATE = false> __device__ __forceinline__ bool wait_ge(Ctl* ctl, const int* p, int target, bool sleepy) {
  unsigned spins = 0;
  unsigned long long t0 = 0;
  while (lds_poll(p) < target) {
    if (sleepy) __builtin_amdgcn_s_sleep(2);
    if ((++spins & 1023u) == 0) {
      bool out;
      if (LATE) { CmxLateBox* const B = ctl_box(ctl); out = B ? late_expired(B, t0) : spins > SPIN_LIMIT; }
      else out = spins > SPIN_LIMIT;
      if (lds_poll(&ctl->abort) || out) {
        lds_publish_store(&ctl->abort, 1);
        return false;
      }
    }
  }
  return true;
}

__device__ __forceinline__ float bcast_lane(float v, int j) {
  return __int_as_float(__builtin_amdgcn_readlane(__float_as_int(v), j));
}

__device__ __forceinline__ float clamp_med3(float x, float mn, float mx) { return __builtin_amdgcn_fmed3f(x, mn, mx); }
__device__ __forceinline__ float clamp_out(float x, float mn, float mx) {
  const float lo = x < mn ? mn : x;
  return x > mx ? mx : lo;
}

__device__ __forceinline__ float4 f4sub_mul(float4 w, float u, float4 x) {
  w.x = fsub(w.x, fmul(u, x.x));
  w.y = fsub(w.y, fmul(u, x.y));
  w.z = fsub(w.z, fmul(u, x.z));
  w.w = fsub(w.w, fmul(u, x.w));
  return w;
}
// ... 236 lines not shown
                                                                     bool prof_on, const CmxVerify& V) {
  uint64_t tprev = __builtin_readcyclecounter();
  uint64_t pacc[3] = {0, 0, 0};
#define TPROF(k) do { if (prof_on) { uint64_t now_ = __builtin_readcyclecounter(); pacc[k] += now_ - tprev; tprev = now_; } } while (0)
  const int k = lane;
  const float cdec = 1.0f - 3.0e-6f;
  const float lr2 = S->lr[CMX_MIXERS - 1];
  const uint16_t* const t_st = S->t_st;
  const uint16_t* const t_sq = S->t_sq;
  uint16_t* const s6 = S->s6;
  uint16_t* const s7 = S->s7;
  int* const x1 = S->x1;
  int* const x2 = S->x2;
  const gptr<uint64_t> row_steps = as_global(S->row_steps);
  float* const w2 = L.w2;
  const gptr<float> rows2 = as_global(S->rows2);
  const gptr<uint64_t> rsteps2 = row_steps + (size_t)(CMX_MIXERS - 1) * CMX_ROWS_PER_MIXER;
  uint32_t cur_row2 = 0xffffffffu;
  uint64_t rs2 = 0, mx2 = S->max_steps[CMX_MIXERS - 1];
  unsigned sj = S->sse_j, spc = S->sse_pc, sffl = S->sse_ffl;
  uint64_t steps_done = 0;
  unsigned long long vdec = 0;
  for (int t = 0; t < nbits; ++t) {
    jitter_stall<JIT>(L.jit, t, 13);
    const float d1f = as_global(decay1)[t];
    if constexpr (VER) vdec += cmx_vmix(CMX_VC_DECAY_GATHER, (uint32_t)t, 0, __float_as_uint(d1f));
    const double d1 = (double)d1f;
    if (k < 13) {
      const unsigned j_ = bcast_u(sj), pc_ = bcast_u(spc), ffl_ = bcast_u(sffl);
      const int a = k % 3, b = k - 9;
      const float* addr;
      if (k < 3) addr = (const float*)(s6 + (size_t)(((((a << 7) + (int)(ffl_ & 127)) << 8) + (int)(pc_ & 255)) * 256 + (int)j_) * 8);
      else if (k < 6) addr = (const float*)(s7 + (size_t)(((((a << 5) + (int)(ffl_ & 31)) << 8) + (int)(pc_ & 255)) * 255 + (j_ ? (int)j_ - 1 : 0)) * 8);
      else if (k < 9) addr = (const float*)(x2 + (((((a << 1) + (int)(ffl_ & 1)) << 8) + (int)(pc_ & 255)) * 256 + (int)j_));
      else addr = (const float*)(x1 + (((((b << 8) + (int)(ffl_ & 255)) << 3) + (int)((pc_ >> 5) & 7)) * 79 + sse_mx1mask((int)j_)));
      touch_line(as_global(addr), L.pfdump + 256 + 256);
    }
    if (!wait_ge<LATE>(L.ctl, &L.ctl->b_in, t + 1, false)) return;
    TPROF(0);
    if (LATE && lane == 0) late_stamp(L.late, 4);
    const float* const in2 = L.h2 + 64 * (t & 1);
    int bit = __float_as_int(in2[49]);
    {
      const uint32_t newrow2 = (uint32_t)__float_as_int(in2[51]);
      if (newrow2 != cur_row2) {
        if (cur_row2 != 0xffffffffu) {
          if (k < 16) gstore4(rows2 + (size_t)cur_row2 * CMX_ROW2_STRIDE + 4 * k, *reinterpret_cast<const float4*>(w2 + 4 * k));
          if (k == 0) rsteps2[cur_row2] = rs2;
        }
        cur_row2 = newrow2;
        if (k < 16) *reinterpret_cast<float4*>(w2 + 4 * k) = gload4(rows2 + (size_t)newrow2 * CMX_ROW2_STRIDE + 4 * k);
        rs2 = rsteps2[newrow2];
        asm volatile("s_waitcnt vmcnt(0) lgkmcnt(0)" ::: "memory");
        __builtin_amdgcn_wave_barrier();
      }
    }
    float u2 = 0.0f;
    int df2 = 0;
    if (k == 0) {
      float acc = 0.0f;
#pragma unroll
      for (int i = 0; i < 12; ++i) {
        const float4 xv = *reinterpret_cast<const float4*>(in2 + 4 * i);
        const float4 wv = *reinterpret_cast<const float4*>(w2 + 4 * i);
        acc = fadd(acc, fmul(xv.x, wv.x)); acc = fadd(acc, fmul(xv.y, wv.y));
        acc = fadd(acc, fmul(xv.z, wv.z)); acc = fadd(acc, fmul(xv.w, wv.w));
      }
      acc = fadd(acc, fmul(in2[48], w2[48]));
      const float p2_ = acc;
      const float sq = cmx_logistic(p2_);
      const int p = (int)(1 + (1 - sq) * 32766);
      const unsigned prq = (unsigned)p >> 11;
      const int a = (prq > 0) + (prq > 14);
      const int b = (prq > 0) + (prq > 7) + (prq > 14);
      const int i6 = ((((a << 7) + (int)(sffl & 127)) << 8) + (int)(spc & 255)) * 256 + (int)sj;
      const int i7 = ((((a << 5) + (int)(sffl & 31)) << 8) + (int)(spc & 255)) * 255 + (sj ? (int)sj - 1 : 0);
      const int im2 = ((((a << 1) + (int)(sffl & 1)) << 8) + (int)(spc & 255)) * 256 + (int)sj;
      const int im1 = ((((b << 8) + (int)(sffl & 255)) << 3) + (int)((spc >> 5) & 7)) * 79 + sse_mx1mask((int)sj);
      U16x8 c6 = load_cell(s6 + (size_t)i6 * 8);
      U16x8 c7 = load_cell(s7 + (size_t)i7 * 8);
      const int w1x = as_global(x1)[im1];
      const int w2x = as_global(x2)[im2];
      SseInterp e6, e7;
      auto ST = [&](int i) -> int { return L.lst ? (int)L.lst[i] : (int)as_global(t_st)[i]; };
      auto SQ = [&](int i) -> int { return L.lsq ? (int)L.lsq[i] : (int)as_global(t_sq)[i]; };
      const int stp = ST(p);
      const int q6 = SQ(sse_extrap(stp, 10240)), q7 = SQ(sse_extrap(stp, 8200));
      const int pp1 = e6.pred(c6, q6);
      const int pp2 = e7.pred(c7, q7);
      const int s0 = sse_extrap(stp, 7935);
      const int s1 = sse_extrap(ST(pp1), 9592);
      const int s4 = sse_extrap(ST(pp2), 7677);
      const int s2 = sse_extrap(sse_mixup(w1x, s0, s1), 8092);
      const int mix1_p = SQ(s2);
      const int s5 = sse_extrap(sse_mixup(w2x, s2, s4), 8202);
      const int mix2_p = SQ(s5);
      float pf = (float)(1 - ((mix2_p - 1) / 32766.0));
      const float lp = in2[50];
      if (lp == 0.0f || lp == 1.0f) pf = lp;
      as_global(p_out)[t] = pf;
      if (LATE) {
        __hip_atomic_store(&L.late.box->p_word[t % CMX_LATE_P_RING], ((unsigned long long)(unsigned)(t + 1) << 32) | (unsigned)__float_as_int(pf), __ATOMIC_RELAXED,
                           __HIP_MEMORY_SCOPE_SYSTEM);
        late_stamp(L.late, 1);
        bit = late_y(L.late, t + 1);
        if (bit < 0) { lds_publish_store(&L.ctl->abort, 1); bit = 0; }
        L.bitring[t & 7] = bit;
        st_rel(&L.ctl->bit_epoch, t + 1);
      }
      e6.update(c6, bit, 106);
      e7.update(c7, bit, 127);
      store_cell_async(s6 + (size_t)i6 * 8, c6);
      store_cell_async(s7 + (size_t)i7 * 8, c7);
      as_global(x1)[im1] = w1x + sse_wdelta(bit, s0, s1, 6202, mix1_p);
      as_global(x2)[im2] = w2x + sse_wdelta(bit, s2, s4, 8320, mix2_p);
      sj += sj + (unsigned)bit;
      if (sj >= 256) {
        sffl = (sffl * 2 + (spc >= 0x40)) & 255;
        spc = sj & 255;
        sj = 1;
      }
      const float decay = (float)(d1 * (1.5 - ((1.0 * (double)rs2) / (double)mx2)));
      u2 = fmul(fmul(decay, lr2), fsub(sq, (float)bit));
      ++rs2;
      if (rs2 > mx2) mx2 = rs2;
      df2 = (rs2 & 1023) == 0;
      if (mix_out) as_global(mix_out)[(size_t)t * CMX_MIXERS + CMX_MIXERS - 1] = p2_;
      ++steps_done;
    }
    if (LATE && lds_poll(&L.ctl->abort)) return;
    TPROF(1);
    u2 = bcast_lane(u2, 0);
    df2 = __builtin_amdgcn_readlane(df2, 0);
    if (k < CMX_IN2) {
      float v = fsub(w2[k], fmul(u2, in2[k]));
      if (df2) v = fmul(v, cdec);
      w2[k] = v;
    }
    asm volatile("s_waitcnt lgkmcnt(0)" ::: "memory");
    __builtin_amdgcn_wave_barrier();
    st_rel(&L.ctl->b_done, t + 1);
    TPROF(2);
    if constexpr (VER) {
      if ((t + 1) % CMX_VERIFY_BLOCK == 0 || t + 1 == nbits) {
        if (lane == 0) as_global(V.rec)[(size_t)(t / CMX_VERIFY_BLOCK) * CMX_VERIFY_REC + CMX_VR_DECAY + 2] = vdec;
        vdec = 0;
      }
    }
  }
  if (prof_on && lane == 0) {
#pragma unroll
    for (int i = 0; i < 3; ++i) S->prof[13 + i] += pacc[i];
  }
#undef TPROF
  if (nbits > 0) {
    asm volatile("s_waitcnt lgkmcnt(0)" ::: "memory");
    __builtin_amdgcn_wave_barrier();
    if (k < 16 && cur_row2 != 0xffffffffu)
      gstore4(rows2 + (size_t)cur_row2 * CMX_ROW2_STRIDE + 4 * k, *reinterpret_cast<const float4*>(w2 + 4 * k));
    if (k == 0) {
      if (cur_row2 != 0xffffffffu) rsteps2[cur_row2] = rs2;
      S->max_steps[CMX_MIXERS - 1] = mx2;
      S->sse_j = sj; S->sse_pc = spc; S->sse_ffl = sffl;
      S->steps = S->steps + steps_done;
    }
  }
}

// ... 579 lines not shown
    GPROF(12);
    if (is0 && mix_out) as_global(mix_out)[(size_t)t * CMX_MIXERS + m] = p_;
#pragma unroll
    for (int j = 0; j < CMX_MIX0; ++j) {
      float oj = bcast_lane(myout, j);
      if (j < m) {
        float v = fsub(ew[j], fmul(uu, oj));
        if (dfl) v = fmul(v, cdec);
        ew[j] = v;
      }
    }
    if (t + 1 < nbits) { d1n = as_global(decay1)[t + 1]; d1_t = t + 1; }
    if (t + 1 < nbits && lds_poll(&L.ctl->scout_epoch) >= t + 2) {
      const BitRec* nx = L.rec + ((t + 1) % L.rr);
      if (is0 && nx->changed[mm]) {
        const gptr<float> r1 = as_global(S->rows0) + ((size_t)mm * CMX_ROWS_PER_MIXER + nx->rowidx[mm]) * CMX_ROW0_STRIDE;
#pragma unroll
        for (int i = 0; i < 7; ++i) ewn[i] = gload4(r1 + CMX_ROW0_EXTRA + 4 * i);
        rsn = (as_global(S->row_steps) + (size_t)mm * CMX_ROWS_PER_MIXER + nx->rowidx[mm])[0];
      }
      pf_t = t + 1;
    }
    GPROF(5);
    if constexpr (VER) {
      if ((t + 1) % CMX_VERIFY_BLOCK == 0 || t + 1 == nbits) {
        if (lane == 0) as_global(V.rec)[(size_t)(t / CMX_VERIFY_BLOCK) * CMX_VERIFY_REC + CMX_VR_DECAY] = vdec;
        vdec = 0;
      }
    }
  }
  if (is0 && nbits > 0) {
    store_row_state();
    S->max_steps[m] = mx;
  }
  if (prof_on && lane == 0) {
#pragma unroll
    for (int i = 0; i < 16; ++i)
      if (i < 6 || i >= 12) S->prof[i] += pacc[i];
  }
#undef GPROF
}

}

template <bool LATE, bool JIT = false, bool VER = false> __device__ __forceinline__ void spec_kernel_body(
    MixState* __restrict__ S, SpecXfer* __restrict__ X, const float* __restrict__ probs, const uint32_t* __restrict__ sel,
    const uint8_t* __restrict__ bits, const float* __restrict__ decay1, int nbits,
    float* __restrict__ p_out, float* __restrict__ mix_out, int mode, const CmxLate& box, const CmxVerify& V = CmxVerify()) {
  static_assert(!(LATE && VER), "verify mode covers the compressor's form only");
  extern __shared__ __attribute__((aligned(16))) float smem[];
  const int tid = threadIdx.x;
  const int wave = __builtin_amdgcn_readfirstlane(tid >> 6), lane = tid & 63;
  int role = (int)blockIdx.x - ((mode >> 8) & 7);
  bool local = false;
  if (role < 0) return;
  if (!(mode & 0x20000) && role > CMX_SPEC_HELPERS) return;
  if (mode & 0x20000) {
    if (!(mode & 0x1000000)) {
      if (((int)blockIdx.x & 7) != ((mode >> 20) & 7)) return;
      role = (int)blockIdx.x >> 3;
    }
    __shared__ int s_local;
    if (tid == 0) {
      unsigned id;
      asm volatile("s_getreg_b32 %0, hwreg(HW_REG_XCC_ID)" : "=s"(id));
      __hip_atomic_store(&X->xcc[role], (id & 15u) + 1u, __ATOMIC_RELAXED, __HIP_MEMORY_SCOPE_AGENT);
    }
    if (wave == 0) {
      unsigned mine = 0, spins = 0;
      bool ok = true;
      for (;;) {
        if (lane <= CMX_SPEC_HELPERS && !mine) mine = ld_u32(&X->xcc[lane]);
        if (__ballot(lane <= CMX_SPEC_HELPERS && !mine) == 0) break;
        __builtin_amdgcn_s_sleep(4);
        if (++spins > (1u << 22) || ld_u32(&X->fail)) { ok = false; break; }
      }
      const unsigned first = (unsigned)__builtin_amdgcn_readlane((int)mine, 0);
      const bool same = __ballot(lane <= CMX_SPEC_HELPERS && mine != first) == 0;
      if (lane == 0) { s_local = ok && same; if (!ok) __hip_atomic_store(&X->fail, 1u, __ATOMIC_RELAXED, __HIP_MEMORY_SCOPE_AGENT); }
    }
    __syncthreads();
    local = s_local != 0 && !(mode & 0x800000);
  }
  if (role > 0) {
    HelperLds* H = reinterpret_cast<HelperLds*>(smem);
    for (int i = tid; i < (int)(sizeof(HelperLds) / 4); i += CMX_SPEC_THREADS) reinterpret_cast<int*>(H)[i] = 0;
    __syncthreads();
    CmxLateBox* const lb = LATE ? box.box : nullptr;
    const bool tol = !LATE && (mode & 0x1000) != 0;
    if (wave < 4) helper_role<LATE, JIT, VER>(S, X, H, nbits, role - 1, wave, lane, tol, lb, local, JIT ? ((mode >> 26) & 15) | 16 : 0, box, probs, V);
    return;
  }
  Lds L;
  L.rec = reinterpret_cast<BitRec*>(smem + 16);
  L.rr = 8; L.lead = 5;
  L.trec = reinterpret_cast<TailRec*>(L.rec + 8);
  L.upd = reinterpret_cast<float*>(L.trec + 2);
  L.dflag = reinterpret_cast<uint32_t*>(L.upd + 32);
  L.in2 = reinterpret_cast<float*>(L.dflag + 32);
  L.ctl = reinterpret_cast<Ctl*>(L.in2 + 64);
  L.pfdump = (unsigned)(size_t)(lds_int*)(reinterpret_cast<int*>(L.ctl) + 16);
  L.w2 = reinterpret_cast<float*>(L.ctl) + 16 + 64;
  L.w1 = L.w2 + 64 + 16 + 64;
  L.exptab = reinterpret_cast<uint64_t*>(L.w1 + 20 * 68);
  L.sdone = reinterpret_cast<int*>(L.exptab + 32);
  uint16_t* lst = reinterpret_cast<uint16_t*>(L.sdone + 8);
  L.lst = lst; L.lsq = lst + 32768;
  L.h2 = reinterpret_cast<float*>(lst + 65536);
  L.bitring = reinterpret_cast<int*>(L.h2 + 128);
  L.late = LATE ? box : CmxLate();
  L.jit = JIT ? ((mode >> 26) & 15) | 16 : 0;
  for (int i = tid; i < 32768; i += CMX_SPEC_THREADS) reinterpret_cast<uint32_t*>(lst)[i] = i < 16384 ? reinterpret_cast<const uint32_t*>(S->t_st)[i] : reinterpret_cast<const uint32_t*>(S->t_sq)[i - 16384];
  if (tid < 32) { L.upd[tid] = 0.0f; L.dflag[tid] = 0; L.exptab[tid] = cmx_exp2f_tab[tid]; }
  if (tid < 8) L.sdone[tid] = 0;
  if (tid < (int)(sizeof(Ctl) / 4)) reinterpret_cast<int*>(L.ctl)[tid] = 0;
  __syncthreads();
  if (LATE && tid == 0) { L.ctl->late_lo = (unsigned)(unsigned long long)box.box; L.ctl->late_hi = (unsigned)((unsigned long long)box.box >> 32); }
  __syncthreads();
  const bool prof = (mode & 4) != 0;
  if (wave == 0) gather_role<LATE, JIT, VER>(S, L, X, decay1, nbits, mix_out, prof, lane, local, V);
  else if (wave == 1) tail_a_role<LATE, JIT, VER>(S, L, decay1, nbits, mix_out, lane, prof && ((mode >> 4) & 4) != 0, V);
  else if (wave == 3) tail_b_role<LATE, JIT, VER>(S, L, decay1, nbits, p_out, mix_out, lane, prof && ((mode >> 4) & 4) != 0, V);
  else if (wave == 2) select_role<LATE, JIT, VER>(S, L, X, sel, probs, nbits, lane, V);
  else if (wave >= 4) stretch_role<LATE, JIT, VER>(S, L, X, probs, bits, nbits, wave - 4, lane, V);
  __syncthreads();
  if (tid == 0 && (L.ctl->abort || ld_u32(&X->fail))) S->error = 1;
}

extern "C" __global__ __launch_bounds__(CMX_SPEC_THREADS) void cmx_mixnet_spec_kernel(
    MixState* __restrict__ S, SpecXfer* __restrict__ X, const float* __restrict__ probs, const uint32_t* __restrict__ sel,
    const uint8_t* __restrict__ bits, const float* __restrict__ decay1, int nbits,
    float* __restrict__ p_out, float* __restrict__ mix_out, int mode) {
  spec_kernel_body<false>(S, X, probs, sel, bits, decay1, nbits, p_out, mix_out, mode, CmxLate());
}
extern "C" __global__ __launch_bounds__(CMX_SPEC_THREADS) void cmx_mixnet_spec_jitter_kernel(
    MixState* __restrict__ S, SpecXfer* __restrict__ X, const float* __restrict__ probs, const uint32_t* __restrict__ sel,
    const uint8_t* __restrict__ bits, const float* __restrict__ decay1, int nbits,
    float* __restrict__ p_out, float* __restrict__ mix_out, int mode) {
  spec_kernel_body<false, true>(S, X, probs, sel, bits, decay1, nbits, p_out, mix_out, mode, CmxLate());
}
extern "C" __global__ __launch_bounds__(CMX_SPEC_THREADS) void cmx_mixnet_spec_late_kernel(
    MixState* __restrict__ S, SpecXfer* __restrict__ X, const float* __restrict__ probs, const uint32_t* __restrict__ sel,
    const float* __restrict__ decay1, int nbits, float* __restrict__ p_out, float* __restrict__ mix_out, int mode, CmxLate box) {
  spec_kernel_body<true>(S, X, probs, sel, nullptr, decay1, nbits, p_out, mix_out, mode, box);
}

extern "C" __global__ __launch_bounds__(CMX_SPEC_THREADS) void cmx_mixnet_spec_verify_kernel(
    MixState* __restrict__ S, SpecXfer* __restrict__ X, const float* __restrict__ probs, const uint32_t* __restrict__ sel,
    const uint8_t* __restrict__ bits, const float* __restrict__ decay1, int nbits,
    float* __restrict__ p_out, float* __restrict__ mix_out, int mode, CmxVerify V) {
  spec_kernel_body<false, false, true>(S, X, probs, sel, bits, decay1, nbits, p_out, mix_out, mode, CmxLate(), V);
}

constexpr int VERIFY_THREADS = 256;
extern "C" __global__ __launch_bounds__(VERIFY_THREADS) void cmx_mixnet_verify_kernel(const MixState* __restrict__ S, const float* __restrict__ probs,
                                                                                     const uint32_t* __restrict__ sel, const uint8_t* __restrict__ bits,
                                                                                     const float* __restrict__ decay1, int nbits, CmxVerify V) {
  const int blk = blockIdx.x, tid = threadIdx.x, lane = tid & 63, wave = tid >> 6;
  const int t0 = blk * CMX_VERIFY_BLOCK;
  const int tn = nbits - t0 < CMX_VERIFY_BLOCK ? nbits - t0 : CMX_VERIFY_BLOCK;
  const gptr<const float> lut = as_global(S->logit_lut);
  unsigned long long e[5] = {0, 0, 0, 0, 0};
  for (int j = tid; j < tn * CMX_IN0; j += VERIFY_THREADS) {
    const int t = t0 + j / CMX_IN0, i = j % CMX_IN0;
    const float pv = as_global(probs)[(size_t)t * CMX_IN0 + i];
    e[0] += cmx_vmix(CMX_VC_ROW, (uint32_t)t, (uint32_t)i, __float_as_uint(pv));
    float p = pv;
    if (p < 1.0e-4f) p = 1.0e-4f;
    else if (p > 1 - 1.0e-4f) p = 1 - 1.0e-4f;
    int idx = (int)(p * 100001.0f);
    if (idx >= 100001) idx = 100000;
    else if (idx < 0) idx = 0;
    e[1] += cmx_vmix(CMX_VC_RING_WRITTEN, (uint32_t)t, (uint32_t)i, __float_as_uint(lut[idx]));
  }
  for (int j = tid; j < tn * CMX_MIXERS; j += VERIFY_THREADS) {
    const int t = t0 + j / CMX_MIXERS, i = j % CMX_MIXERS;
    e[3] += cmx_vmix(CMX_VC_SEL, (uint32_t)t, (uint32_t)i, as_global(sel)[(size_t)t * CMX_MIXERS + i]);
  }
  if (tid < tn) {
    e[2] = cmx_vmix(CMX_VC_BIT, (uint32_t)(t0 + tid), 0, (uint32_t)as_global(bits)[t0 + tid]);
    e[4] = cmx_vmix(CMX_VC_DECAY_GATHER, (uint32_t)(t0 + tid), 0, __float_as_uint(as_global(decay1)[t0 + tid]));
  }
  __shared__ unsigned long long part[VERIFY_THREADS / 64][5];
#pragma unroll
  for (int k = 0; k < 5; ++k) {
    const unsigned long long v = wave_sum_u64(e[k]);
    if (lane == 0) part[wave][k] = v;
  }
  __syncthreads();
  if (tid != 0) return;
  unsigned long long x[5];
#pragma unroll
  for (int k = 0; k < 5; ++k) x[k] = part[0][k] + part[1][k] + part[2][k] + part[3][k];
  const gptr<const unsigned long long> rec = as_global((const unsigned long long*)V.rec) + (size_t)blk * CMX_VERIFY_REC;
  unsigned long long n = 0, first = ~0ull;
  auto check = [&](unsigned long long got, unsigned long long want, uint32_t cls, uint32_t m) {
    if (got == want) return;
    ++n;
    const unsigned long long k = cmx_vkey((uint32_t)blk, cls, m, 0, 0);
    if (k < first) first = k;
  };
  check(rec[CMX_VR_ROW] + rec[CMX_VR_ROW + 1] + rec[CMX_VR_ROW + 2] + rec[CMX_VR_ROW + 3], x[0], CMX_VC_ROW, 0);
  check(rec[CMX_VR_BIT] + rec[CMX_VR_BIT + 1] + rec[CMX_VR_BIT + 2] + rec[CMX_VR_BIT + 3], x[2], CMX_VC_BIT, 0);
  check(rec[CMX_VR_SEL], x[3], CMX_VC_SEL, 0);
  check(rec[CMX_VR_DECAY], x[4], CMX_VC_DECAY_GATHER, 0);
  check(rec[CMX_VR_DECAY + 1], x[4], CMX_VC_DECAY_TAIL_A, 0);
  check(rec[CMX_VR_DECAY + 2], x[4], CMX_VC_DECAY_TAIL_B, 0);
  check(rec[CMX_VR_RINGW] + rec[CMX_VR_RINGW + 1] + rec[CMX_VR_RINGW + 2] + rec[CMX_VR_RINGW + 3], x[1], CMX_VC_RING_WRITTEN, 0);
  for (int m = 0; m < CMX_MIX0; ++m) {
    const int b = CMX_VR_RINGR + 4 * m;
// ... 34 lines not shown
```

cmix_amd/csrc/mixnet_state.h:

```cpp
#ifndef CMX_MIXNET_STATE_H
#define CMX_MIXNET_STATE_H
#include <stdint.h>

#define CMX_IN0 2078
#define CMX_IN1 29
#define CMX_IN2 49
#define CMX_MIX0 26
#define CMX_MIX1 20
#define CMX_MIXERS 47
#define CMX_AUX 12

#define CMX_ROW_LIMIT 10000u
#define CMX_ROWS_PER_MIXER 10001u
#define CMX_MAP_SLOTS 32768u

#define CMX_ROW0_STRIDE 2112
#define CMX_ROW0_EXTRA 2080
#define CMX_ROW1_STRIDE 64
#define CMX_ROW1_EXTRA 32
#define CMX_ROW2_STRIDE 64

#define CMX_SM6_VOL (3 * 128 * 256 * 256)
#define CMX_MIX1_VOL (4 * 256 * 8 * 79)
#define CMX_SM7_VOL (3 * 32 * 256 * 255)
#define CMX_MIX2_VOL (3 * 2 * 256 * 256)

struct MixState {
  const float* logit_lut;
  const uint16_t* t_st;
  const uint16_t* t_sq;
  float stretch_min, stretch_max;
  float lr[CMX_MIXERS];

  float* rows0;
  float* rows1;
  float* rows2;
  uint64_t* row_steps;
  uint32_t* map_keys;
  uint32_t* map_vals;
  uint32_t n_rows[CMX_MIXERS + 1];
  uint64_t max_steps[CMX_MIXERS + 1];
  uint64_t steps;

  uint16_t* s6;
  uint16_t* s7;
  int* x1;
  int* x2;
  uint32_t sse_j, sse_pc, sse_ffl;

  float fwd_p[CMX_MIXERS + 1];
  float fwd_out0[32];
  float fwd_in2[64];

  int error;
  int pad_;
  uint64_t prof[16];
};

#define CMX_SPEC_RING 8
#define CMX_SPEC_XS 2112
#define CMX_SPEC_HELPERS CMX_MIX0
#define CMX_SPEC_THREADS 512
#define CMX_MIXNET_XCD_DEFAULT (-1)
struct SpecXfer {
  unsigned scout_epoch;
  unsigned fail;
  unsigned sel_epoch;
  unsigned pad0[13];
  unsigned xcc[32];
  unsigned long long u[32];
  unsigned long long sum[32];
  unsigned rowidx[CMX_SPEC_RING][32];
  unsigned changed[CMX_SPEC_RING][32];
  float xs[CMX_SPEC_RING][CMX_SPEC_XS];
  unsigned long long stat[8];
};
#define CMX_SPEC_HEADER_BYTES (64 + 128 + 2 * 32 * 8)
#define CMX_SPEC_LDS_BYTES 147456

#endif
```

cmix_amd/engine.py:

```python
import ctypes as C
import os

import numpy as np

HERE = os.path.dirname(os.path.abspath(__file__))
LIB_PATH = os.path.join(HERE, "lib", "libcmixamd.so")

N_INPUTS, N_MIXERS = 2078, 47
PIPELINE_SLOTS = 8


class CmxError(RuntimeError):
    pass


_lib = None


def lib():
    global _lib
    if _lib is None:
        if not os.path.exists(LIB_PATH):
            raise CmxError(f"{LIB_PATH} is missing: run `python -m cmix_amd.build` "
                           "(there is no non-HIP fallback)")
        try:
            import torch
        except ImportError:
            pass
        L = C.CDLL(LIB_PATH)
        L.cmx_last_error.restype = C.c_char_p
        L.cmx_version.restype = C.c_char_p
        L.cmx_p8stage_create.restype = C.c_void_p
        L.cmx_p8stage_create.argtypes = [C.c_int]
        L.cmx_p8stage_destroy.argtypes = [C.c_void_p]
        L.cmx_p8stage_run.argtypes = [C.c_void_p, C.c_void_p, C.c_size_t, C.c_void_p, C.c_size_t, C.c_void_p]
        L.cmx_p8stage_sync.argtypes = [C.c_void_p]
        L.cmx_p8stage_set_generator_counter.argtypes = [C.c_void_p, C.c_uint32]
        L.cmx_fxcm_create.restype = C.c_void_p
        L.cmx_fxcm_create.argtypes = [C.c_char_p, C.c_int]
        L.cmx_fxcm_destroy.argtypes = [C.c_void_p]
        L.cmx_fxcm_run.argtypes = [C.c_void_p, C.c_void_p, C.c_void_p, C.c_size_t, C.c_void_p, C.c_void_p, C.c_void_p, C.c_size_t, C.c_void_p]
        L.cmx_fxcm_sync.argtypes = [C.c_void_p]
        L.cmx_fxcm_failed.argtypes = [C.c_void_p]
        L.cmx_mixnet_create.restype = C.c_void_p
        L.cmx_mixnet_create.argtypes = [C.c_int]
        L.cmx_mixnet_destroy.argtypes = [C.c_void_p]
        L.cmx_mixnet_run.argtypes = [C.c_void_p, C.c_void_p, C.c_void_p, C.c_void_p, C.c_size_t,
                                     C.c_void_p, C.c_void_p, C.c_void_p]
        L.cmx_mixnet_predict.restype = C.c_float
        L.cmx_mixnet_predict.argtypes = [C.c_void_p, C.c_void_p, C.c_void_p]
        L.cmx_mixnet_perceive.argtypes = [C.c_void_p, C.c_int]
        L.cmx_mixnet_sync.argtypes = [C.c_void_p]
        L.cmx_mixnet_bits_done.argtypes = [C.c_void_p, C.c_void_p]
        L.cmx_mixnet_profile.argtypes = [C.c_void_p, C.c_int, C.c_void_p]
        L.cmx_mixnet_last_kernel_ms.argtypes = [C.c_void_p, C.c_void_p]
        L.cmx_mixnet_spec_stats.argtypes = [C.c_void_p, C.c_void_p]
        L.cmx_lstm_create.restype = C.c_void_p
        L.cmx_lstm_create.argtypes = [C.c_void_p, C.c_int, C.c_int]
        L.cmx_lstm_destroy.argtypes = [C.c_void_p]
        L.cmx_lstm_vocab_size.argtypes = [C.c_void_p]
        L.cmx_lstm_set_tolerance.argtypes = [C.c_void_p, C.c_int]
        L.cmx_lstm_run.argtypes = [C.c_void_p, C.c_void_p, C.c_void_p, C.c_size_t, C.c_void_p, C.c_void_p,
                                   C.c_size_t, C.c_void_p, C.c_void_p]
        L.cmx_bytemodel_bits_run.argtypes = [C.c_int, C.c_void_p, C.c_void_p, C.c_void_p, C.c_size_t,
                                             C.c_void_p, C.c_size_t, C.c_void_p, C.c_void_p]
        L.cmx_lstm_get_gate_weights.argtypes = [C.c_void_p, C.c_int, C.c_int, C.c_void_p]
        L.cmx_lstm_gate_rowlen.argtypes = [C.c_void_p, C.c_int]
        L.cmx_lstm_failed.argtypes = [C.c_void_p]
        L.cmx_glibc_rand_selftest.argtypes = [C.c_uint32, C.c_int, C.c_void_p]
        L.cmx_ctxmodels_create.restype = C.c_void_p
        L.cmx_ctxmodels_create.argtypes = [C.c_void_p, C.c_int]
        L.cmx_ctxmodels_destroy.argtypes = [C.c_void_p]
        L.cmx_ctxmodels_run.argtypes = [C.c_void_p, C.c_void_p, C.c_size_t, C.c_void_p, C.c_size_t, C.c_void_p,
                                        C.c_void_p]
        L.cmx_ctxmodels_pretrain.argtypes = [C.c_void_p, C.c_void_p, C.c_size_t, C.c_void_p]
        L.cmx_ctxmodels_sync.argtypes = [C.c_void_p]
        L.cmx_ctxmodels_get_manager.argtypes = [C.c_void_p, C.c_void_p, C.c_void_p, C.c_void_p]
        L.cmx_ppmd_create.restype = C.c_void_p
        L.cmx_ppmd_create.argtypes = [C.c_void_p]
        L.cmx_ppmd_create_ex.restype = C.c_void_p
        L.cmx_ppmd_create_ex.argtypes = [C.c_void_p, C.c_int, C.c_int]
        L.cmx_ppmd_destroy.argtypes = [C.c_void_p]
        L.cmx_ppmd_run.argtypes = [C.c_void_p, C.c_void_p, C.c_size_t, C.c_void_p]
        L.cmx_pipeline_create.restype = C.c_void_p
        L.cmx_pipeline_create.argtypes = [C.c_void_p, C.c_int, C.c_size_t]
        L.cmx_pipeline_destroy.argtypes = [C.c_void_p]
        L.cmx_pipeline_submit.argtypes = [C.c_void_p, C.c_void_p, C.c_size_t, C.c_void_p, C.c_void_p]
        L.cmx_create.restype = C.c_void_p
        L.cmx_create.argtypes = [C.c_void_p, C.c_char_p, C.c_int]
        L.cmx_destroy.argtypes = [C.c_void_p]
        L.cmx_predict.restype = C.c_float
        L.cmx_predict.argtypes = [C.c_void_p]
        L.cmx_perceive.argtypes = [C.c_void_p, C.c_int]
        L.cmx_pretrain.argtypes = [C.c_void_p, C.c_int]
        L.cmx_set_model_outputs.argtypes = [C.c_void_p, C.c_void_p]
        L.cmx_get_lstm_hint.argtypes = [C.c_void_p, C.c_void_p, C.c_void_p]
        L.cmx_stage_input.argtypes = [C.c_void_p, C.c_void_p, C.c_size_t]
        L.cmx_mode.argtypes = [C.c_void_p, C.c_void_p]
        L.cmx_debug_last_row.restype = C.c_void_p
        L.cmx_debug_last_row.argtypes = [C.c_void_p]
        L.cmx_ctxmodels_debug_slow_bytes.argtypes = [C.c_void_p, C.c_void_p]
        L.cmx_ctxmodels_peek.argtypes = [C.c_void_p, C.c_void_p, C.c_int, C.c_void_p, C.c_size_t, C.c_void_p, C.c_void_p]
        L.cmx_encoder_create.restype = C.c_void_p
        L.cmx_encoder_destroy.argtypes = [C.c_void_p]
        L.cmx_encoder_encode_bits.argtypes = [C.c_void_p, C.c_void_p, C.c_void_p, C.c_size_t]
        L.cmx_encoder_encode_bytes.argtypes = [C.c_void_p, C.c_void_p, C.c_void_p, C.c_size_t]
        L.cmx_encoder_flush.argtypes = [C.c_void_p]
        L.cmx_encoder_size.restype = C.c_size_t
        L.cmx_encoder_size.argtypes = [C.c_void_p]
        L.cmx_encoder_data.restype = C.c_void_p
        L.cmx_encoder_data.argtypes = [C.c_void_p]
        L.cmx_decoder_create.restype = C.c_void_p
        L.cmx_decoder_create.argtypes = [C.c_void_p, C.c_size_t]
        L.cmx_decoder_destroy.argtypes = [C.c_void_p]
        L.cmx_decoder_decode.argtypes = [C.c_void_p, C.c_float]
        L.cmx_decoder_decode_bits.argtypes = [C.c_void_p, C.c_void_p, C.c_size_t, C.c_void_p]
        L.cmx_header_write.restype = C.c_size_t
        L.cmx_header_write.argtypes = [C.c_uint64, C.c_void_p, C.c_int, C.c_void_p]
        L.cmx_header_read.restype = C.c_size_t
        L.cmx_header_read.argtypes = [C.c_void_p, C.c_size_t, C.c_void_p, C.c_void_p, C.c_void_p]
        L.cmx_pipeline_begin.argtypes = [C.c_void_p, C.c_void_p, C.c_size_t, C.c_void_p]
        L.cmx_pipeline_hints.argtypes = [C.c_void_p, C.c_void_p, C.c_void_p]
        L.cmx_pipeline_finish.argtypes = [C.c_void_p, C.c_void_p, C.c_void_p]
        L.cmx_pipeline_stage_totals.argtypes = [C.c_void_p, C.c_void_p, C.c_void_p, C.c_int]
        L.cmx_pipeline_pretrain.argtypes = [C.c_void_p, C.c_void_p, C.c_size_t]
        L.cmx_pipeline_sync.argtypes = [C.c_void_p]
        L.cmx_pipeline_enable_fxcm.argtypes = [C.c_void_p, C.c_char_p]
        L.cmx_pipeline_fxcm_enabled.argtypes = [C.c_void_p]
        L.cmx_pipeline_finish_cols.argtypes = [C.c_void_p, C.c_void_p, C.c_int, C.c_int, C.c_void_p]
        L.cmx_pipeline_fxcm_total_ms.argtypes = [C.c_void_p, C.c_void_p]
        L.cmx_pipeline_enable_paq8.argtypes = [C.c_void_p]
        L.cmx_pipeline_wait.argtypes = [C.c_void_p, C.c_uint64]
        L.cmx_pipeline_debug_mix_out.argtypes = [C.c_void_p, C.c_void_p, C.c_uint64]
        L.cmx_pipeline_paq8_total_ms.argtypes = [C.c_void_p, C.c_void_p]
        L.cmx_pipeline_host_ms.argtypes = [C.c_void_p, C.c_void_p]
        L.cmx_pipeline_paq8_role_ms.argtypes = [C.c_void_p, C.c_void_p, C.c_void_p]
        L.cmx_pipeline_last_stage_ms.argtypes = [C.c_void_p, C.c_void_p]
        L.cmx_probe_libm.argtypes = [C.c_int, C.c_int, C.c_void_p, C.c_void_p, C.c_size_t]
        L.cmx_pipeline_set_tolerance.argtypes = [C.c_void_p, C.c_int]
# ... 77 lines not shown
        return _verify_report(lib().cmx_mixnet_verify_report, self.h)

    def debug_verify_perturb(self, cls, bit, index, xor_mask):
        cls = VERIFY_CLASS.get(cls, cls)
        if lib().cmx_mixnet_debug_verify_perturb(self.h, int(cls), int(bit), int(index), int(xor_mask)):
            raise CmxError(last_error())

    def close(self):
        if getattr(self, "h", None):
            lib().cmx_mixnet_destroy(self.h)
            self.h = None

    def __del__(self):
        try:
            self.close()
        except Exception:
            pass

    def run(self, probs, sel, bits, p_out=None, mix_out=None, stream=None):
        import torch
        T = int(bits.numel())
        assert probs.is_cuda and sel.is_cuda and bits.is_cuda
        assert probs.dtype == torch.float32 and probs.is_contiguous() and probs.numel() == T * N_INPUTS
        assert sel.dtype == torch.int32 and sel.is_contiguous() and sel.numel() == T * N_MIXERS
        assert bits.dtype == torch.uint8 and bits.is_contiguous()
        if p_out is None:
            p_out = torch.empty(T, dtype=torch.float32, device=probs.device)
        if stream is None:
            stream = torch.cuda.current_stream(probs.device).cuda_stream
        rc = lib().cmx_mixnet_run(self.h, probs.data_ptr(), sel.data_ptr(), bits.data_ptr(), T,
                                  p_out.data_ptr(), mix_out.data_ptr() if mix_out is not None else None,
                                  C.c_void_p(stream))
        if rc:
            raise CmxError(last_error())
        return p_out

    def predict(self, probs, sel):
        probs = np.ascontiguousarray(probs, np.float32)
        sel = np.ascontiguousarray(sel, np.uint32)
        assert probs.size == N_INPUTS and sel.size == N_MIXERS
        p = lib().cmx_mixnet_predict(self.h, probs.ctypes.data, sel.ctypes.data)
        if p < 0:
            raise CmxError(last_error())
        return np.float32(p)

    def perceive(self, bit):
        if lib().cmx_mixnet_perceive(self.h, int(bit)):
            raise CmxError(last_error())

    def sync(self):
        if lib().cmx_mixnet_sync(self.h):
            raise CmxError(last_error())

    def bits_done(self):
        v = C.c_uint64(0)
        if lib().cmx_mixnet_bits_done(self.h, C.byref(v)):
            raise CmxError(last_error())
        return v.value

    def profile(self, enable=True):
        out = (C.c_uint64 * 16)()
        if lib().cmx_mixnet_profile(self.h, int(enable), out):
            raise CmxError(last_error())
        return list(out)

    def last_kernel_ms(self):
        v = C.c_float(0)
        if lib().cmx_mixnet_last_kernel_ms(self.h, C.byref(v)):
            raise CmxError(last_error())
        return v.value

    def debug_set_steps(self, steps):
        lib().cmx_mixnet_debug_set_steps.argtypes = [C.c_void_p, C.c_uint64]
        if lib().cmx_mixnet_debug_set_steps(self.h, int(steps)):
            raise CmxError(last_error())

    def spec_stats(self):
        out = (C.c_uint64 * 5)()
        if lib().cmx_mixnet_spec_stats(self.h, out):
            raise CmxError(last_error())
        v = list(out)
        return {"segments": v[0], "hits": v[1], "reruns": v[2:5], "hit_rate": (v[1] / v[0]) if v[0] else None}


class Lstm:
    SKIP_RAND = 31

    def __init__(self, vocab, device=0, skip_rand=SKIP_RAND):
        vocab = np.ascontiguousarray(vocab, np.uint8)
        assert vocab.size == 256
        self.h = lib().cmx_lstm_create(vocab.ctypes.data, skip_rand, device)
        if not self.h:
            raise CmxError(last_error())
        self.V = lib().cmx_lstm_vocab_size(self.h)

    def set_tolerance(self, on=True):
        if lib().cmx_lstm_set_tolerance(self.h, 1 if on else 0):
            raise CmxError(last_error())

    def close(self):
        if getattr(self, "h", None):
            lib().cmx_lstm_destroy(self.h)
            self.h = None

    def __del__(self):
        try:
            self.close()
        except Exception:
            pass

    def run(self, in_probs, data, want_bits=True, stream=None, layer0=None, out=None):
        import torch
        N = int(data.numel())
        assert in_probs.is_cuda and in_probs.dtype == torch.float32 and in_probs.is_contiguous()
        assert in_probs.numel() == N * 256 and data.dtype == torch.uint8 and data.is_contiguous()
        if out is None:
            out = torch.empty((N, 256), dtype=torch.float32, device=in_probs.device)
        bp, bp_ptr, stride = None, None, 1
        if layer0 is not None:
            assert layer0.dtype == torch.float32 and layer0.is_contiguous() and layer0.shape == (8 * N, N_INPUTS)
            bp_ptr, stride = layer0.data_ptr() + 4 * (N_INPUTS - 1), N_INPUTS
        elif want_bits:
            bp = torch.empty((N, 8), dtype=torch.float32, device=in_probs.device)
            bp_ptr = bp.data_ptr()
        bx = torch.empty((N, 8), dtype=torch.int32, device=in_probs.device) if bp_ptr else None
        if stream is None:
            stream = torch.cuda.current_stream(in_probs.device).cuda_stream
        rc = lib().cmx_lstm_run(self.h, in_probs.data_ptr(), data.data_ptr(), N, out.data_ptr(),
                                bp_ptr, stride, bx.data_ptr() if bx is not None else None, C.c_void_p(stream))
        if rc:
            raise CmxError(last_error())
        return out, bp, bx

    def gate_weights(self, layer, gate):
        n = lib().cmx_lstm_gate_rowlen(self.h, layer)
        out = np.empty((200, n), np.float32)
        if lib().cmx_lstm_get_gate_weights(self.h, layer, gate, out.ctypes.data):
            raise CmxError("cmx_lstm_get_gate_weights failed")
        return out


SMALL_COLS = [0, 1, 2] + list(range(2025, 2076))


class CtxModels:

    def __init__(self, vocab, device=0):
        vocab = np.ascontiguousarray(vocab, np.uint8)
        assert vocab.size == 256
        self.h = lib().cmx_ctxmodels_create(vocab.ctypes.data, device)
        if not self.h:
            raise CmxError(last_error())

    def close(self):
        if getattr(self, "h", None):
            lib().cmx_ctxmodels_destroy(self.h)
            self.h = None

    def __del__(self):
        try:
            self.close()
        except Exception:
            pass

    def run(self, data, probs=None, sel=None, stream=None):
        import torch
# ... 530 lines not shown
```

include/cmix_amd.h:

```cpp
#ifndef CMIX_AMD_H
#define CMIX_AMD_H

#include <stddef.h>
#include <stdint.h>

#ifdef __cplusplus
extern "C" {
#endif

#define CMX_N_INPUTS 2078
#define CMX_N_MIXERS 47
#define CMX_N_MIX0 26
#define CMX_N_MIX1 20
#define CMX_AUX_MIXER 12

const char* cmx_last_error(void);
int cmx_device_count(void);
const char* cmx_version(void);
void* cmx_device_alloc(int device, size_t bytes);
void cmx_device_free(int device, void* p);
void* cmx_host_alloc(size_t bytes);
void cmx_host_free(void* p);
int cmx_copy_to_host(int device, void* dst, const void* d_src, size_t bytes);

typedef struct cmx_engine cmx_t;
cmx_t* cmx_create(const uint8_t vocab[256], const char* dict_path, int device);
float cmx_predict(cmx_t*);
int cmx_perceive(cmx_t*, int bit);
int cmx_pretrain(cmx_t*, int bit);
int cmx_decode_stream(cmx_t*, const uint8_t* code, size_t code_len, uint8_t* out, size_t nbytes);
int cmx_set_model_outputs(cmx_t*, const float cols_3_to_2024[2022]);
int cmx_get_lstm_hint(cmx_t*, int* lstmpr, int* lstmex);
const float* cmx_debug_last_row(cmx_t*);
int cmx_stage_input(cmx_t*, const uint8_t* bytes, size_t n);
int cmx_mode(cmx_t*, int* chunks_in_flight);
int cmx_set_verify(cmx_t*, int on);
int cmx_verify_report(cmx_t*, uint64_t out[8]);
void cmx_destroy(cmx_t*);

typedef struct cmx_mixnet cmx_mixnet_t;
cmx_mixnet_t* cmx_mixnet_create(int device);
void cmx_mixnet_destroy(cmx_mixnet_t*);

int cmx_mixnet_set_tolerance(cmx_mixnet_t*, int on);
const int* cmx_mixnet_error_flag(cmx_mixnet_t*);
int cmx_mixnet_mode(cmx_mixnet_t*);
int cmx_mixnet_set_upload_stream(cmx_mixnet_t*, void* stream);
int cmx_mixnet_run(cmx_mixnet_t*, const float* d_probs, const uint32_t* d_sel,
                   const uint8_t* d_bits, size_t nbits, float* d_p_out, float* d_mix_out,
                   void* stream);

float cmx_mixnet_predict(cmx_mixnet_t*, const float* probs2078, const uint32_t* sel47);
int cmx_mixnet_perceive(cmx_mixnet_t*, int bit);

int cmx_mixnet_predict_async(cmx_mixnet_t*, const float* d_probs2078, const uint32_t* d_sel47, float* d_p, void* stream);
int cmx_mixnet_perceive_async(cmx_mixnet_t*, int bit, void* stream);

int cmx_mixnet_sync(cmx_mixnet_t*);

int cmx_mixnet_bits_done(const cmx_mixnet_t*, uint64_t* out);
int cmx_mixnet_profile(cmx_mixnet_t*, int enable, uint64_t* out16);
int cmx_mixnet_last_kernel_ms(cmx_mixnet_t*, float* ms);
int cmx_mixnet_spec_stats(cmx_mixnet_t*, uint64_t out[5]);
int cmx_mixnet_debug_set_steps(cmx_mixnet_t*, uint64_t steps);
int cmx_mixnet_set_verify(cmx_mixnet_t*, int on);
int cmx_mixnet_verify_on(cmx_mixnet_t*);
int cmx_mixnet_verify_report(cmx_mixnet_t*, uint64_t out[8]);
const unsigned long long* cmx_mixnet_verify_record(cmx_mixnet_t*);
int cmx_mixnet_debug_verify_perturb(cmx_mixnet_t*, int cls, uint64_t bit, uint64_t index, uint32_t xor_mask);

typedef struct cmx_lstm cmx_lstm_t;
cmx_lstm_t* cmx_lstm_create(const uint8_t vocab[256], int skip_rand, int device);
void cmx_lstm_destroy(cmx_lstm_t*);
int cmx_lstm_vocab_size(const cmx_lstm_t*);
int cmx_lstm_run(cmx_lstm_t*, const float* d_in_probs, const uint8_t* d_bytes, size_t nbytes,
                 float* d_out_probs, float* d_bit_p, size_t bit_p_stride, int* d_bit_ex, void* stream);
int cmx_bytemodel_bits_run(int device, const float* d_dist0, const float* d_dist_rest,
                           const uint8_t* d_bytes, size_t nbytes, float* d_bit_p, size_t bit_p_stride,
                           int* d_bit_ex, void* stream);
int cmx_bytemodel_bit_run(int device, const float* d_dist, const uint8_t* d_byte, int k, float* d_bit_p,
                          size_t bit_p_stride, int* d_bit_ex, float* d_p_copy, void* stream);
int cmx_lstm_get_gate_weights(cmx_lstm_t*, int layer, int gate, float* out_host);
int cmx_lstm_gate_rowlen(const cmx_lstm_t*, int layer);
int cmx_lstm_failed(cmx_lstm_t*);
int cmx_lstm_set_tolerance(cmx_lstm_t*, int on);
const unsigned* cmx_lstm_fail_flag(cmx_lstm_t*);
int cmx_glibc_rand_selftest(uint32_t seed, int n, int* out);

typedef struct cmx_ctxmodels cmx_ctxmodels_t;
cmx_ctxmodels_t* cmx_ctxmodels_create(const uint8_t vocab[256], int device);
void cmx_ctxmodels_destroy(cmx_ctxmodels_t*);
int cmx_ctxmodels_run(cmx_ctxmodels_t*, const uint8_t* d_bytes, size_t nbytes, float* d_probs, size_t pstride,
                      uint32_t* d_sel, void* stream);
int cmx_ctxmodels_peek(cmx_ctxmodels_t*, const uint8_t* d_byte, int bit_index ,
                       float* d_probs8, size_t probs_stride, uint32_t* d_sel8, void* stream);
int cmx_ctxmodels_pretrain(cmx_ctxmodels_t*, const uint8_t* d_bytes, size_t nbytes, void* stream);
int cmx_ctxmodels_debug_slow_bytes(cmx_ctxmodels_t*, uint64_t out2[2]);
int cmx_ctxmodels_debug_set_history(cmx_ctxmodels_t*, uint64_t pos, const uint8_t* tail, uint64_t n);
int cmx_ctxmodels_sync(cmx_ctxmodels_t*);
int cmx_ctxmodels_get_manager(cmx_ctxmodels_t*, uint64_t* regs25, uint64_t* ctx54, uint64_t* bitctx8);

typedef struct cmx_fxcm cmx_fxcm_t;
cmx_fxcm_t* cmx_fxcm_create(const char* dictionary_path, int device);
void cmx_fxcm_destroy(cmx_fxcm_t*);
int cmx_fxcm_run(cmx_fxcm_t*, const uint8_t* bytes, const uint8_t* d_bytes, size_t nbytes, const int16_t* d_lstmpr, const uint8_t* d_lstmex,
                 float* d_probs, size_t pstride, void* stream);
int cmx_fxcm_sync(cmx_fxcm_t*);
int cmx_fxcm_failed(cmx_fxcm_t*);
const unsigned* cmx_fxcm_fail_flag(cmx_fxcm_t*);
int cmx_fxcm_set_upload_stream(cmx_fxcm_t*, void* stream);
int cmx_fxcm_profile(cmx_fxcm_t*, unsigned long long out128[128]);

typedef struct cmx_encoder cmx_encoder_t;
typedef struct cmx_decoder cmx_decoder_t;
cmx_encoder_t* cmx_encoder_create(void);
void cmx_encoder_destroy(cmx_encoder_t*);
int cmx_encoder_encode_bits(cmx_encoder_t*, const float* p, const uint8_t* bits, size_t nbits);
int cmx_encoder_encode_bytes(cmx_encoder_t*, const float* p , const uint8_t* bytes, size_t nbytes);
int cmx_encoder_flush(cmx_encoder_t*);
size_t cmx_encoder_size(const cmx_encoder_t*);
const uint8_t* cmx_encoder_data(const cmx_encoder_t*);
cmx_decoder_t* cmx_decoder_create(const uint8_t* code, size_t len);
void cmx_decoder_destroy(cmx_decoder_t*);
int cmx_decoder_decode(cmx_decoder_t*, float p);
int cmx_decoder_decode_bits(cmx_decoder_t*, const float* p, size_t nbits, uint8_t* bits_out);
#define CMX_HEADER_MAX 37
#define CMX_MIN_VOCAB_FILE_SIZE 10000
size_t cmx_header_write(uint64_t length, const uint8_t vocab[256], int dictionary_used, uint8_t out[CMX_HEADER_MAX]);
size_t cmx_header_read(const uint8_t* in, size_t len, uint64_t* length, int* dictionary_used, uint8_t vocab[256]);

typedef struct cmx_ppmd cmx_ppmd_t;
cmx_ppmd_t* cmx_ppmd_create(const uint8_t vocab[256]);
cmx_ppmd_t* cmx_ppmd_create_ex(const uint8_t vocab[256], int order, int memory_mb);
void cmx_ppmd_destroy(cmx_ppmd_t*);
int cmx_ppmd_run(cmx_ppmd_t*, const uint8_t* bytes, size_t nbytes, float* out_probs);

#define CMX_PIPELINE_SLOTS 8
#define CMX_MAX_HW_QUEUES 32
int cmx_hw_queues(int device);
int cmx_prewarm(int device, const char* dictionary_path, int with_fxcm);

typedef struct cmx_pipeline cmx_pipeline_t;
cmx_pipeline_t* cmx_pipeline_create(const uint8_t vocab[256], int device, size_t max_chunk_bytes);
void cmx_pipeline_destroy(cmx_pipeline_t*);
int cmx_pipeline_stage_overlap(cmx_pipeline_t*);
int cmx_pipeline_submit(cmx_pipeline_t*, const uint8_t* bytes, size_t n, float* d_layer0, float* d_p_out);
// ... 86 lines not shown
```

Baseline: 17830.

## Pin mixnet spec kernel to a free XCD, shrink compressor LDS, drop LSTM XCD avoidance

The compressor form of the spec kernel no longer stages the SSE stretch/squash tables in LDS and reads them from global memory instead. This shrinks its dynamic LDS to at most 16 KB so it can share a compute unit with a large LSTM workgroup. Each mixnet handle now claims a free XCD by default through a per-device allocator (the decoder's late path stays unpinned), and the LSTM kernels drop their remapping that kept blocks off the mixnet's XCD. The aim is to give the serial mixnet its own XCD with better locality while the LSTM gets the full grid. The risks are slower global table lookups in the mixnet inner loop and contention if placement interacts badly.

```diff
diff --git a/cmix_amd/csrc/cmx_api.hip b/cmix_amd/csrc/cmx_api.hip
--- a/cmix_amd/csrc/cmx_api.hip
+++ b/cmix_amd/csrc/cmx_api.hip
@@ -23,6 +23,7 @@
 extern "C" __global__ void cmx_mixnet_spec_late_kernel(MixState*, SpecXfer*, const float*, const uint32_t*, const float*, int, float*, float*, int, CmxLate);
 extern "C" __global__ void cmx_mixnet_spec_verify_kernel(MixState*, SpecXfer*, const float*, const uint32_t*, const uint8_t*, const float*, int, float*, float*, int,
                                                          CmxVerify);
+extern "C" unsigned cmx_mixnet_spec_lds_bytes(int late);
 extern "C" __global__ void cmx_mixnet_verify_kernel(const MixState*, const float*, const uint32_t*, const uint8_t*, const float*, int, CmxVerify);
 extern "C" __global__ void cmx_mixnet_verify_fold_kernel(CmxVerifyHdr*, unsigned long long, int);
 extern "C" __global__ void cmx_mixnet_verify_xor_kernel(void*, int, unsigned);
@@ -123,6 +124,8 @@
   int rotate = 0;
   int jitter = 0;
   int xcd = -1;
+  bool xcd_asked = false;
+  bool xcd_forced = false;
   bool tolerance = false;
   SpecXfer* d_xfer = nullptr;
   float* d_late_p = nullptr; size_t late_p_cap = 0;
@@ -203,8 +206,27 @@
   return 0;
 }
 
+namespace {
+std::mutex g_xcd_mu;
+constexpr int XCD_MAX_DEV = 64;
+unsigned g_xcd_used[XCD_MAX_DEV];
+int xcd_take(int dev) {
+  if (dev < 0 || dev >= XCD_MAX_DEV) return -1;
+  std::lock_guard<std::mutex> g(g_xcd_mu);
+  for (int k = 7; k >= 0; --k)
+    if (!(g_xcd_used[dev] >> k & 1u)) { g_xcd_used[dev] |= 1u << k; return k; }
+  return -1;
+}
+void xcd_give(int dev, int k) {
+  if (dev < 0 || dev >= XCD_MAX_DEV || k < 0 || k >= 8) return;
+  std::lock_guard<std::mutex> g(g_xcd_mu);
+  g_xcd_used[dev] &= ~(1u << k);
+}
+}
+
 void cmx_mixnet_destroy(cmx_mixnet_t* h) {
   if (!h) return;
+  if (!h->xcd_forced) xcd_give(h->device, h->xcd);
   hipSetDevice(h->device);
   hipDeviceSynchronize();
   for (void* p : h->allocs) hipFree(p);
@@ -297,7 +319,7 @@
   bool attr_ok = true;
   for (const void* k : {(const void*)cmx_mixnet_spec_kernel, (const void*)cmx_mixnet_spec_jitter_kernel, (const void*)cmx_mixnet_spec_late_kernel,
                         (const void*)cmx_mixnet_spec_verify_kernel})
-    attr_ok = attr_ok && hipFuncSetAttribute(k, hipFuncAttributeMaxDynamicSharedMemorySize, CMX_SPEC_LDS_BYTES) == hipSuccess;
+    attr_ok = attr_ok && hipFuncSetAttribute(k, hipFuncAttributeMaxDynamicSharedMemorySize, (int)cmx_mixnet_spec_lds_bytes(k == (const void*)cmx_mixnet_spec_late_kernel)) == hipSuccess;
   if (!h->d_xfer || !attr_ok) {
     set_err("cmx_mixnet_create: hand-off area / kernel attribute (spec kernel) failed");
     cmx_mixnet_destroy(h);
@@ -306,7 +328,8 @@
   { const char* v = getenv("CMX_MIXNET_DBG"); h->dbg = v ? atoi(v) : 0; }
   { const char* v = getenv("CMX_MIXNET_JITTER"); h->jitter = v ? atoi(v) & 15 : 0; }
   { const char* v = getenv("CMX_MIXNET_ROTATE"); h->rotate = v && v[0] == '1'; }
-  { const char* v = getenv("CMX_MIXNET_XCD"); h->xcd = v ? atoi(v) : CMX_MIXNET_XCD_DEFAULT; if (h->xcd > 7) h->xcd = -1; }
+  if (const char* v = getenv("CMX_MIXNET_XCD")) { h->xcd = atoi(v); if (h->xcd < 0 || h->xcd > 7) h->xcd = -1; h->xcd_forced = true; }
+  else if (h->rotate || getenv("CMX_MIXNET_PADGRID")) h->xcd_forced = true;
   hipEventCreate(&h->ev0);
   hipEventCreate(&h->ev1);
   for (int i = 0; i < CMX_PIPELINE_SLOTS; ++i) { hipEventCreateWithFlags(&h->ev_decay[i], hipEventDisableTiming); hipEventCreateWithFlags(&h->ev_kdone[i], hipEventDisableTiming); }
@@ -335,6 +358,17 @@
   h->allocs.push_back(p);
   h->d_decay = (float*)p;
   h->decay_cap = cap;
+  return 0;
+}
+
+int cmx_mixnet_placement(cmx_mixnet_t* h, int out[2]) {
+  const int fail_value = 1;
+  if (!h || !out) { set_err("cmx_mixnet_placement: bad argument"); return 1; }
+  HIP_OK(hipSetDevice(h->device));
+  HIP_OK(hipDeviceSynchronize());
+  unsigned long long form = 0;
+  HIP_OK(hipMemcpy(&form, (char*)h->d_xfer + offsetof(SpecXfer, stat) + 5 * 8, 8, hipMemcpyDeviceToHost));
+  out[0] = h->xcd; out[1] = (int)form;
   return 0;
 }
 
@@ -597,14 +631,18 @@
   h->decay_used[slot] = true;
   HIP_OK(hipEventRecord(h->ev0, st));
   HIP_OK(hipMemsetAsync(h->d_xfer, 0, CMX_SPEC_HEADER_BYTES, st));
+  const bool late = box && box->box;
+  if (!late && !h->xcd_forced && !h->xcd_asked) { h->xcd = xcd_take(h->device); h->xcd_asked = true; }
+  const int xcd = late && !h->xcd_forced ? -1 : h->xcd;
   const bool cumask = cmx_cumask_on() != 0;
-  const int rot = h->rotate && h->xcd < 0 ? (int)((h->runs * 3) & 7) : 0;
-  const int kmode = 3 | (rot << 8) | (h->profile ? 4 : 0) | ((h->dbg & 15) << 4) | (h->tolerance ? 0x1000 : 0) | (h->xcd >= 0 ? 0x20000 | ((h->xcd & 7) << 20) : 0) |
+  const int rot = h->rotate && xcd < 0 ? (int)((h->runs * 3) & 7) : 0;
+  const int kmode = 3 | (rot << 8) | (h->profile ? 4 : 0) | ((h->dbg & 15) << 4) | (h->tolerance ? 0x1000 : 0) | (xcd >= 0 ? 0x20000 | ((xcd & 7) << 20) : 0) |
                     (getenv("CMX_MIXNET_XCD_NOLOCAL") ? 0x800000 : 0) | (cumask ? 0x1000000 : 0) | (h->jitter ? 0x2000000 | ((h->jitter & 15) << 26) : 0);
   static const bool padgrid = getenv("CMX_MIXNET_PADGRID") != nullptr;
-  const unsigned grid = (1 + CMX_SPEC_HELPERS) * ((h->xcd >= 0 && !cumask) || padgrid ? 8 : 1) + (unsigned)rot;
-  if (box && box->box)
-    hipLaunchKernelGGL(cmx_mixnet_spec_late_kernel, dim3(grid), dim3(CMX_SPEC_THREADS), CMX_SPEC_LDS_BYTES, st,
+  const unsigned grid = (1 + CMX_SPEC_HELPERS) * ((xcd >= 0 && !cumask) || padgrid ? 8 : 1) + (unsigned)rot;
+  const unsigned lds = cmx_mixnet_spec_lds_bytes(late);
+  if (late)
+    hipLaunchKernelGGL(cmx_mixnet_spec_late_kernel, dim3(grid), dim3(CMX_SPEC_THREADS), lds, st,
                        h->d_state, h->d_xfer, d_probs, d_sel, dd, (int)nbits, d_p_out, d_mix_out, kmode, *box);
   else if (h->verify) {
     HIP_OK(hipMemsetAsync(h->d_vhdr, 0, CMX_VERIFY_CLEAR_BYTES, st));
@@ -620,7 +658,7 @@
       hipLaunchKernelGGL(cmx_mixnet_verify_xor_kernel, dim3(1), dim3(64), 0, st, (void*)(h->h_state.rows0 + p.bit * CMX_ROW0_STRIDE + p.index), 4, p.mask);
     const bool ring = p.cls == CMX_VC_RING_WRITTEN || p.cls == CMX_VC_RING_READ;
     const CmxVerify V = {h->d_vrec, h->d_vseg, h->d_vhdr, ring ? (int)p.bit : -1, ring ? (int)p.index : 0, ring ? p.mask : 0u};
-    hipLaunchKernelGGL(cmx_mixnet_spec_verify_kernel, dim3(grid), dim3(CMX_SPEC_THREADS), CMX_SPEC_LDS_BYTES, st,
+    hipLaunchKernelGGL(cmx_mixnet_spec_verify_kernel, dim3(grid), dim3(CMX_SPEC_THREADS), lds, st,
                        h->d_state, h->d_xfer, d_probs, d_sel, d_bits, dd, (int)nbits, d_p_out, d_mix_out, kmode, V);
     HIP_OK(hipGetLastError());
     if (pw) hipLaunchKernelGGL(cmx_mixnet_verify_xor_kernel, dim3(1), dim3(64), 0, st, pw, pbytes, p.mask);
@@ -628,7 +666,7 @@
     if (pw) hipLaunchKernelGGL(cmx_mixnet_verify_xor_kernel, dim3(1), dim3(64), 0, st, pw, pbytes, p.mask);
     hipLaunchKernelGGL(cmx_mixnet_verify_fold_kernel, dim3(1), dim3(64), 0, st, h->d_vhdr, (unsigned long long)h->bits_done, (int)nbits);
   } else {
-    hipLaunchKernelGGL(h->jitter ? cmx_mixnet_spec_jitter_kernel : cmx_mixnet_spec_kernel, dim3(grid), dim3(CMX_SPEC_THREADS), CMX_SPEC_LDS_BYTES, st,
+    hipLaunchKernelGGL(h->jitter ? cmx_mixnet_spec_jitter_kernel : cmx_mixnet_spec_kernel, dim3(grid), dim3(CMX_SPEC_THREADS), lds, st,
                        h->d_state, h->d_xfer, d_probs, d_sel, d_bits, dd, (int)nbits, d_p_out, d_mix_out, kmode);
   }
   HIP_OK(hipGetLastError());
diff --git a/cmix_amd/csrc/lstm_api.hip b/cmix_amd/csrc/lstm_api.hip
--- a/cmix_amd/csrc/lstm_api.hip
+++ b/cmix_amd/csrc/lstm_api.hip
@@ -8,7 +8,6 @@
 #include <vector>
 
 #include "../../include/cmix_amd.h"
-#include "mixnet_state.h"
 #include "lstm_state.h"
 #include "cmx_late.h"
 #include "cmx_glibc_rand.h"
@@ -56,6 +55,8 @@
   for (int i = 0; i < n; ++i) out[i] = g.next();
   return 0;
 }
+
+unsigned cmx_lstm_block_lds_bytes(int V, int which) { return (unsigned)(which ? lstm_bp_lds_bytes() : lstm_fb_lds_bytes(V)); }
 
 cmx_lstm_t* cmx_lstm_create(const uint8_t vocab[256], int skip_rand, int device) {
   int ndev = cmx_device_count();
@@ -80,7 +81,6 @@
   S.rowlen[1] = S.insz[1] + V;
   S.lr = 0.03f;
   { const char* v = getenv("CMX_LSTM_XCD"); S.xcd = v ? atoi(v) : -1; }
-  { const char* v = getenv("CMX_LSTM_AVOID_XCD"); if (!v) v = getenv("CMX_MIXNET_XCD"); S.avoid_xcd = v ? atoi(v) : CMX_MIXNET_XCD_DEFAULT; if (S.avoid_xcd > 7) S.avoid_xcd = -1; }
   bool fail = false;
   auto dallocf = [&](size_t count, const float* init) -> float* {
     void* p = nullptr;
@@ -179,13 +179,8 @@
   S.logit_ring = dallocf((size_t)LSTM_H * LSTM_VP, nullptr);
   S.bp_pub = dallocf((size_t)2 * LSTM_H * 2 * LSTM_C, nullptr);
   {
-    const size_t nq1 = (size_t)(S.insz[1] + 3) / 4;
-    const size_t gate = nq1 * LSTM_FB_R * 16 + (836 + 3 * LSTM_C + 4 + 256) * 4;
-    const size_t ro = (size_t)(V + LSTM_FB_GO - 1) / LSTM_FB_GO, rp = ro | 1;
-    const size_t outl = (size_t)((LSTM_NH + 3) / 4) * rp * 16 + (2 * 404 + 256 + 256 + 36 + 36 + 4) * 4;
-    h->fb_lds = gate > outl ? gate : outl;
-    h->bp_lds = (size_t)9 * 50 * LSTM_BP_J * 16 +
-                ((size_t)3 * 256 * LSTM_BP_J + 3 * 256 + 3 * LSTM_C + 3 * LSTM_C + 4 + 6 * LSTM_BP_J) * 4;
+    h->fb_lds = lstm_fb_lds_bytes(V);
+    h->bp_lds = lstm_bp_lds_bytes();
     if (hipFuncSetAttribute((const void*)cmx_lstm_fwdblk, hipFuncAttributeMaxDynamicSharedMemorySize, (int)h->fb_lds) != hipSuccess ||
         hipFuncSetAttribute((const void*)cmx_lstm_fwdblk_late, hipFuncAttributeMaxDynamicSharedMemorySize, (int)h->fb_lds) != hipSuccess ||
         hipFuncSetAttribute((const void*)cmx_lstm_bpttblk, hipFuncAttributeMaxDynamicSharedMemorySize, (int)h->bp_lds) != hipSuccess)
@@ -227,15 +222,15 @@
     if (e == 0) {
       hipLaunchKernelGGL(cmx_lstm_prep, dim3(1), dim3(256), 0, st, S, d_in_probs + n * 256, d_bytes, n, e, -1);
       if (!sync_reset()) { cmx_set_err("cmx_lstm_run: hipMemsetAsync failed"); return 1; }
-      hipLaunchKernelGGL(cmx_lstm_bpttblk, dim3(lstm_grid_for_roles(LSTM_BP_G, S.avoid_xcd)), dim3(LSTM_BP_THREADS), h->bp_lds, st, S);
+      hipLaunchKernelGGL(cmx_lstm_bpttblk, dim3(LSTM_BP_G), dim3(LSTM_BP_THREADS), h->bp_lds, st, S);
       if (h->tolerance) hipLaunchKernelGGL(cmx_lstm_bptt_acc_mfma, dim3((S.rowlen[1] + 15) / 16, (LSTM_C + 15) / 16, 6), dim3(64), 0, st, S, us, -1);
-      else { const int gx = (S.rowlen[1] + 63) / 64, gy = LSTM_C / 4; hipLaunchKernelGGL(cmx_lstm_bptt_acc, dim3(lstm_grid_for_roles(gx * gy * 6, S.avoid_xcd)), dim3(64, 4), 0, st, S, us, -1, gx, gy); }
+      else { const int gx = (S.rowlen[1] + 63) / 64, gy = LSTM_C / 4; hipLaunchKernelGGL(cmx_lstm_bptt_acc, dim3(gx * gy * 6), dim3(64, 4), 0, st, S, us, -1, gx, gy); }
       hipLaunchKernelGGL(cmx_lstm_bptt_gb, dim3(6), dim3(256), 0, st, S, us, -1);
     }
     const size_t left = nbytes - n;
     const int cnt = (int)(left < (size_t)(LSTM_H - e) ? left : (size_t)(LSTM_H - e));
     if (!sync_reset()) { cmx_set_err("cmx_lstm_run: hipMemsetAsync failed"); return 1; }
-    hipLaunchKernelGGL(cmx_lstm_fwdblk, dim3(lstm_grid_for_roles(2 * LSTM_FB_GL + LSTM_FB_GO, S.avoid_xcd)), dim3(LSTM_FB_THREADS), h->fb_lds, st, S, d_bytes,
+    hipLaunchKernelGGL(cmx_lstm_fwdblk, dim3(2 * LSTM_FB_GL + LSTM_FB_GO), dim3(LSTM_FB_THREADS), h->fb_lds, st, S, d_bytes,
                        d_in_probs, d_out_probs, n, cnt, e, hc);
     h->hc ^= 1;
     h->bytes_done += cnt;
@@ -265,14 +260,14 @@
     const int us = (int)(h->bptt_rounds < LSTM_UPDATE_LIMIT ? h->bptt_rounds : LSTM_UPDATE_LIMIT);
     hipLaunchKernelGGL(cmx_lstm_prep, dim3(1), dim3(256), 0, st, S, h_ppmd + (b0 + 1) * 256, h_bytes, b0, e, -1);
     if (!sync_reset()) { cmx_set_err("cmx_lstm_run_late: hipMemsetAsync failed"); return -1; }
-    hipLaunchKernelGGL(cmx_lstm_bpttblk, dim3(lstm_grid_for_roles(LSTM_BP_G, S.avoid_xcd)), dim3(LSTM_BP_THREADS), h->bp_lds, st, S);
-    { const int gx = (S.rowlen[1] + 63) / 64, gy = LSTM_C / 4; hipLaunchKernelGGL(cmx_lstm_bptt_acc, dim3(lstm_grid_for_roles(gx * gy * 6, S.avoid_xcd)), dim3(64, 4), 0, st, S, us, -1, gx, gy); }
+    hipLaunchKernelGGL(cmx_lstm_bpttblk, dim3(LSTM_BP_G), dim3(LSTM_BP_THREADS), h->bp_lds, st, S);
+    { const int gx = (S.rowlen[1] + 63) / 64, gy = LSTM_C / 4; hipLaunchKernelGGL(cmx_lstm_bptt_acc, dim3(gx * gy * 6), dim3(64, 4), 0, st, S, us, -1, gx, gy); }
     hipLaunchKernelGGL(cmx_lstm_bptt_gb, dim3(6), dim3(256), 0, st, S, us, -1);
   }
   const size_t left = nchunk - b0;
   const int cnt = (int)(left < (size_t)(LSTM_H - e) ? left : (size_t)(LSTM_H - e));
   if (!sync_reset()) { cmx_set_err("cmx_lstm_run_late: hipMemsetAsync failed"); return -1; }
-  hipLaunchKernelGGL(cmx_lstm_fwdblk_late, dim3(lstm_grid_for_roles(2 * LSTM_FB_GL + LSTM_FB_GO, S.avoid_xcd)), dim3(LSTM_FB_THREADS), h->fb_lds, st, S, *(const CmxLate*)late_box,
+  hipLaunchKernelGGL(cmx_lstm_fwdblk_late, dim3(2 * LSTM_FB_GL + LSTM_FB_GO), dim3(LSTM_FB_THREADS), h->fb_lds, st, S, *(const CmxLate*)late_box,
                      d_ppmd, h_ppmd, d_out, (int)b0, cnt, e, hc, (int)nchunk);
   h->hc ^= 1;
   h->bytes_done += cnt;
diff --git a/cmix_amd/csrc/lstm_block.hip b/cmix_amd/csrc/lstm_block.hip
--- a/cmix_amd/csrc/lstm_block.hip
+++ b/cmix_amd/csrc/lstm_block.hip
@@ -387,8 +387,8 @@
   extern __shared__ float4 fb_lds[];
   FbArgs A;
   A.bytes = bytes; A.in_probs = in_probs; A.out_probs = out_probs; A.n0 = n0; A.cnt = cnt; A.e0 = e0; A.hc = hc;
-  const int b = lstm_role_of_block((int)blockIdx.x, P.avoid_xcd);
-  if (b < 0 || b >= 2 * GL + GO) return;
+  const int b = (int)blockIdx.x;
+  if (b >= 2 * GL + GO) return;
   A.late = CmxLate(); A.d_ppmd = nullptr; A.h_ppmd = nullptr; A.nchunk = 0;
   if (b < GL) fb_gate_wg<false>(&P, A, 0, b, reinterpret_cast<float*>(fb_lds));
   else if (b < 2 * GL) fb_gate_wg<false>(&P, A, 1, b - GL, reinterpret_cast<float*>(fb_lds));
@@ -401,8 +401,8 @@
   FbArgs A;
   A.bytes = nullptr; A.in_probs = nullptr; A.out_probs = out_probs; A.n0 = (size_t)b0; A.cnt = cnt; A.e0 = e0; A.hc = hc;
   A.late = late; A.d_ppmd = d_ppmd; A.h_ppmd = h_ppmd; A.nchunk = nchunk;
-  const int b = lstm_role_of_block((int)blockIdx.x, P.avoid_xcd);
-  if (b < 0 || b >= 2 * GL + GO) return;
+  const int b = (int)blockIdx.x;
+  if (b >= 2 * GL + GO) return;
   if (b < GL) fb_gate_wg<true>(&P, A, 0, b, reinterpret_cast<float*>(fb_lds));
   else if (b < 2 * GL) fb_gate_wg<true>(&P, A, 1, b - GL, reinterpret_cast<float*>(fb_lds));
   else fb_out_wg<true>(&P, A, b - 2 * GL, reinterpret_cast<float*>(fb_lds));
@@ -420,8 +420,8 @@
   extern __shared__ float4 bp_lds[];
   const LstmState* S = &P;
   LstmSync* Y = S->sync;
-  const int tid = threadIdx.x, V = S->V, b = lstm_role_of_block((int)blockIdx.x, P.avoid_xcd), j0 = b * J;
-  if (b < 0 || b >= GB) return;
+  const int tid = threadIdx.x, V = S->V, b = (int)blockIdx.x, j0 = b * J;
+  if (b >= GB) return;
   const bool lead = b == 0;
   float4* Wb = bp_lds;
   float* olb = reinterpret_cast<float*>(Wb + 9 * 50 * J);
diff --git a/cmix_amd/csrc/lstm_kernels.hip b/cmix_amd/csrc/lstm_kernels.hip
--- a/cmix_amd/csrc/lstm_kernels.hip
+++ b/cmix_amd/csrc/lstm_kernels.hip
@@ -44,8 +44,8 @@
   __shared__ float es[H][4];
   __shared__ float ins[H][64];
   __shared__ unsigned sym[H];
-  const int role = lstm_role_of_block((int)blockIdx.x, P.avoid_xcd);
-  if (role < 0 || role >= gx * gy * 6) return;
+  const int role = (int)blockIdx.x;
+  if (role >= gx * gy * 6) return;
   const int bx = role % gx, by = (role / gx) % gy, bz = role / (gx * gy);
   const int layer = bz / 3, g = bz % 3;
   const int V = S->V, rl = S->rowlen[layer], insz = S->insz[layer];
diff --git a/cmix_amd/csrc/lstm_state.h b/cmix_amd/csrc/lstm_state.h
--- a/cmix_amd/csrc/lstm_state.h
+++ b/cmix_amd/csrc/lstm_state.h
@@ -1,5 +1,6 @@
 #ifndef CMX_LSTM_STATE_H
 #define CMX_LSTM_STATE_H
+#include <stddef.h>
 #include <stdint.h>
 
 #define LSTM_C 200
@@ -44,7 +45,6 @@
   unsigned char vocab[256];
   float lr;
   int xcd;
-  int avoid_xcd;
 
   float* W[LSTM_L][3];
   float* WT[LSTM_L][3];
@@ -79,20 +79,15 @@
 };
 
 #if defined(__HIPCC__) || defined(__cplusplus)
-static inline
-#if defined(__HIPCC__)
-__host__ __device__
-#endif
-int lstm_role_of_block(int b, int avoid) {
-  if (avoid < 0) return b;
-  if ((b & 7) == avoid) return -1;
-  return b - (b >= avoid ? (b - avoid) / 8 + 1 : 0);
+static inline size_t lstm_fb_lds_bytes(int V) {
+  const size_t nq1 = (size_t)(V + 1 + 2 * LSTM_C + 3) / 4;
+  const size_t gate = nq1 * LSTM_FB_R * 16 + (836 + 3 * LSTM_C + 4 + 256) * 4;
+  const size_t ro = (size_t)(V + LSTM_FB_GO - 1) / LSTM_FB_GO, rp = ro | 1;
+  const size_t outl = (size_t)((LSTM_NH + 3) / 4) * rp * 16 + (2 * 404 + 256 + 256 + 36 + 36 + 4) * 4;
+  return gate > outl ? gate : outl;
 }
-static inline int lstm_grid_for_roles(int n, int avoid) {
-  if (avoid < 0) return n;
-  int g = n;
-  while (lstm_role_of_block(g - 1, avoid) < n - 1) ++g;
-  return g;
+static inline size_t lstm_bp_lds_bytes(void) {
+  return (size_t)9 * 50 * LSTM_BP_J * 16 + ((size_t)3 * 256 * LSTM_BP_J + 3 * 256 + 3 * LSTM_C + 3 * LSTM_C + 4 + 6 * LSTM_BP_J) * 4;
 }
 static inline
 #if defined(__HIPCC__)
diff --git a/cmix_amd/csrc/mixnet_chunk.hip b/cmix_amd/csrc/mixnet_chunk.hip
--- a/cmix_amd/csrc/mixnet_chunk.hip
+++ b/cmix_amd/csrc/mixnet_chunk.hip
@@ -60,6 +60,26 @@
   CmxLate late;
   int jit;
 };
+
+template <bool TABLES> struct MainLds {
+  static constexpr size_t rec = 16 * 4;
+  static constexpr size_t trec = rec + 8 * sizeof(BitRec);
+  static constexpr size_t upd = trec + 2 * sizeof(TailRec);
+  static constexpr size_t dflag = upd + 32 * 4;
+  static constexpr size_t in2 = dflag + 32 * 4;
+  static constexpr size_t ctl = in2 + 64 * 4;
+  static constexpr size_t pfdump = ctl + 16 * 4;
+  static constexpr size_t w2 = pfdump + 256;
+  static constexpr size_t w1 = w2 + (64 + 16 + 64) * 4;
+  static constexpr size_t exptab = w1 + 20 * 68 * 4;
+  static constexpr size_t sdone = exptab + 32 * 8;
+  static constexpr size_t tables = sdone + 8 * 4;
+  static constexpr size_t h2 = tables + (TABLES ? 2 * 32768 * 2 : 0);
+  static constexpr size_t bitring = h2 + 128 * 4;
+  static constexpr size_t end = bitring + 8 * 4;
+};
+static_assert(sizeof(Ctl) <= 16 * 4 && MainLds<false>::exptab % 8 == 0 && MainLds<true>::tables % 4 == 0 && MainLds<true>::h2 % 16 == 0 && MainLds<false>::h2 % 16 == 0,
+              "main workgroup's LDS layout");
 
 template <bool JIT> __device__ __forceinline__ void jitter_stall(int jit, int t, int who) {
   if constexpr (!JIT) return;
@@ -462,8 +482,8 @@
       const int w1x = as_global(x1)[im1];
       const int w2x = as_global(x2)[im2];
       SseInterp e6, e7;
-      auto ST = [&](int i) -> int { return L.lst ? (int)L.lst[i] : (int)as_global(t_st)[i]; };
-      auto SQ = [&](int i) -> int { return L.lsq ? (int)L.lsq[i] : (int)as_global(t_sq)[i]; };
+      auto ST = [&](int i) -> int { if constexpr (LATE) return (int)L.lst[i]; else return (int)as_global(t_st)[i]; };
+      auto SQ = [&](int i) -> int { if constexpr (LATE) return (int)L.lsq[i]; else return (int)as_global(t_sq)[i]; };
       const int stp = ST(p);
       const int q6 = SQ(sse_extrap(stp, 10240)), q7 = SQ(sse_extrap(stp, 8200));
       const int pp1 = e6.pred(c6, q6);
@@ -1209,6 +1229,7 @@
     __syncthreads();
     local = s_local != 0 && !(mode & 0x800000);
   }
+  if (role == 0 && tid == 0) X->stat[5] = !(mode & 0x20000) ? 0u : local ? 2u : 1u;
   if (role > 0) {
     HelperLds* H = reinterpret_cast<HelperLds*>(smem);
     for (int i = tid; i < (int)(sizeof(HelperLds) / 4); i += CMX_SPEC_THREADS) reinterpret_cast<int*>(H)[i] = 0;
@@ -1218,26 +1239,29 @@
     if (wave < 4) helper_role<LATE, JIT, VER>(S, X, H, nbits, role - 1, wave, lane, tol, lb, local, JIT ? ((mode >> 26) & 15) | 16 : 0, box, probs, V);
     return;
   }
+  using M = MainLds<LATE>;
+  char* const sm = reinterpret_cast<char*>(smem);
   Lds L;
-  L.rec = reinterpret_cast<BitRec*>(smem + 16);
+  L.rec = reinterpret_cast<BitRec*>(sm + M::rec);
   L.rr = 8; L.lead = 5;
-  L.trec = reinterpret_cast<TailRec*>(L.rec + 8);
-  L.upd = reinterpret_cast<float*>(L.trec + 2);
-  L.dflag = reinterpret_cast<uint32_t*>(L.upd + 32);
-  L.in2 = reinterpret_cast<float*>(L.dflag + 32);
-  L.ctl = reinterpret_cast<Ctl*>(L.in2 + 64);
-  L.pfdump = (unsigned)(size_t)(lds_int*)(reinterpret_cast<int*>(L.ctl) + 16);
-  L.w2 = reinterpret_cast<float*>(L.ctl) + 16 + 64;
-  L.w1 = L.w2 + 64 + 16 + 64;
-  L.exptab = reinterpret_cast<uint64_t*>(L.w1 + 20 * 68);
-  L.sdone = reinterpret_cast<int*>(L.exptab + 32);
-  uint16_t* lst = reinterpret_cast<uint16_t*>(L.sdone + 8);
-  L.lst = lst; L.lsq = lst + 32768;
-  L.h2 = reinterpret_cast<float*>(lst + 65536);
-  L.bitring = reinterpret_cast<int*>(L.h2 + 128);
+  L.trec = reinterpret_cast<TailRec*>(sm + M::trec);
+  L.upd = reinterpret_cast<float*>(sm + M::upd);
+  L.dflag = reinterpret_cast<uint32_t*>(sm + M::dflag);
+  L.in2 = reinterpret_cast<float*>(sm + M::in2);
+  L.ctl = reinterpret_cast<Ctl*>(sm + M::ctl);
+  L.pfdump = (unsigned)(size_t)(lds_int*)(sm + M::pfdump);
+  L.w2 = reinterpret_cast<float*>(sm + M::w2);
+  L.w1 = reinterpret_cast<float*>(sm + M::w1);
+  L.exptab = reinterpret_cast<uint64_t*>(sm + M::exptab);
+  L.sdone = reinterpret_cast<int*>(sm + M::sdone);
+  uint16_t* const lst = reinterpret_cast<uint16_t*>(sm + M::tables);
+  L.lst = LATE ? lst : nullptr; L.lsq = LATE ? lst + 32768 : nullptr;
+  L.h2 = reinterpret_cast<float*>(sm + M::h2);
+  L.bitring = reinterpret_cast<int*>(sm + M::bitring);
   L.late = LATE ? box : CmxLate();
   L.jit = JIT ? ((mode >> 26) & 15) | 16 : 0;
-  for (int i = tid; i < 32768; i += CMX_SPEC_THREADS) reinterpret_cast<uint32_t*>(lst)[i] = i < 16384 ? reinterpret_cast<const uint32_t*>(S->t_st)[i] : reinterpret_cast<const uint32_t*>(S->t_sq)[i - 16384];
+  if constexpr (LATE)
+    for (int i = tid; i < 32768; i += CMX_SPEC_THREADS) reinterpret_cast<uint32_t*>(lst)[i] = i < 16384 ? reinterpret_cast<const uint32_t*>(S->t_st)[i] : reinterpret_cast<const uint32_t*>(S->t_sq)[i - 16384];
   if (tid < 32) { L.upd[tid] = 0.0f; L.dflag[tid] = 0; L.exptab[tid] = cmx_exp2f_tab[tid]; }
   if (tid < 8) L.sdone[tid] = 0;
   if (tid < (int)(sizeof(Ctl) / 4)) reinterpret_cast<int*>(L.ctl)[tid] = 0;
@@ -1253,6 +1277,11 @@
   __syncthreads();
   if (tid == 0 && (L.ctl->abort || ld_u32(&X->fail))) S->error = 1;
 }
+
+static_assert(MainLds<true>::end <= CMX_SPEC_LDS_BYTES && sizeof(HelperLds) <= MainLds<true>::end, "the decoder's form keeps its LDS size");
+constexpr size_t kSpecLdsCompress = ((MainLds<false>::end > sizeof(HelperLds) ? MainLds<false>::end : sizeof(HelperLds)) + 255) / 256 * 256;
+static_assert(kSpecLdsCompress <= 16384, "the compressor's form must fit beside another stage's 132 KB workgroup on a compute unit (160 KB)");
+extern "C" unsigned cmx_mixnet_spec_lds_bytes(int late) { return late ? (unsigned)CMX_SPEC_LDS_BYTES : (unsigned)kSpecLdsCompress; }
 
 extern "C" __global__ __launch_bounds__(CMX_SPEC_THREADS) void cmx_mixnet_spec_kernel(
     MixState* __restrict__ S, SpecXfer* __restrict__ X, const float* __restrict__ probs, const uint32_t* __restrict__ sel,
diff --git a/cmix_amd/csrc/mixnet_state.h b/cmix_amd/csrc/mixnet_state.h
--- a/cmix_amd/csrc/mixnet_state.h
+++ b/cmix_amd/csrc/mixnet_state.h
@@ -61,7 +61,6 @@
 #define CMX_SPEC_XS 2112
 #define CMX_SPEC_HELPERS CMX_MIX0
 #define CMX_SPEC_THREADS 512
-#define CMX_MIXNET_XCD_DEFAULT (-1)
 struct SpecXfer {
   unsigned scout_epoch;
   unsigned fail;
diff --git a/cmix_amd/engine.py b/cmix_amd/engine.py
--- a/cmix_amd/engine.py
+++ b/cmix_amd/engine.py
@@ -55,6 +55,11 @@
         L.cmx_mixnet_profile.argtypes = [C.c_void_p, C.c_int, C.c_void_p]
         L.cmx_mixnet_last_kernel_ms.argtypes = [C.c_void_p, C.c_void_p]
         L.cmx_mixnet_spec_stats.argtypes = [C.c_void_p, C.c_void_p]
+        L.cmx_mixnet_placement.argtypes = [C.c_void_p, C.c_void_p]
+        L.cmx_mixnet_spec_lds_bytes.restype = C.c_uint
+        L.cmx_mixnet_spec_lds_bytes.argtypes = [C.c_int]
+        L.cmx_lstm_block_lds_bytes.restype = C.c_uint
+        L.cmx_lstm_block_lds_bytes.argtypes = [C.c_int, C.c_int]
         L.cmx_lstm_create.restype = C.c_void_p
         L.cmx_lstm_create.argtypes = [C.c_void_p, C.c_int, C.c_int]
         L.cmx_lstm_destroy.argtypes = [C.c_void_p]
@@ -298,6 +303,12 @@
         v = list(out)
         return {"segments": v[0], "hits": v[1], "reruns": v[2:5], "hit_rate": (v[1] / v[0]) if v[0] else None}
 
+    def placement(self):
+        out = (C.c_int * 2)()
+        if lib().cmx_mixnet_placement(self.h, out):
+            raise CmxError(last_error())
+        return out[0], out[1]
+
 
 class Lstm:
     SKIP_RAND = 31
diff --git a/include/cmix_amd.h b/include/cmix_amd.h
--- a/include/cmix_amd.h
+++ b/include/cmix_amd.h
@@ -62,6 +62,9 @@
 int cmx_mixnet_profile(cmx_mixnet_t*, int enable, uint64_t* out16);
 int cmx_mixnet_last_kernel_ms(cmx_mixnet_t*, float* ms);
 int cmx_mixnet_spec_stats(cmx_mixnet_t*, uint64_t out[5]);
+int cmx_mixnet_placement(cmx_mixnet_t*, int out[2]);
+unsigned cmx_mixnet_spec_lds_bytes(int late);
+unsigned cmx_lstm_block_lds_bytes(int V, int which);
 int cmx_mixnet_debug_set_steps(cmx_mixnet_t*, uint64_t steps);
 int cmx_mixnet_set_verify(cmx_mixnet_t*, int on);
 int cmx_mixnet_verify_on(cmx_mixnet_t*);
```

Result: faster. 19460, median of 6 (+9.2%).
